# eichenberger/stereo-svo-slam

Hardware: AMD Instinct MI355X
Metric: tracked_frames_per_sec (higher is better)
Workload: dtype f32

## Files before the change

### include/svo_hip.h

```cpp
#ifndef SVO_HIP_H
#define SVO_HIP_H

#include <stddef.h>

#include "svo_types.h"

#ifdef __cplusplus
extern "C" {
#endif

enum {
    SVO_OK = 0,
    SVO_ERR_INVALID = -1,
    SVO_ERR_HIP = -2,
    SVO_ERR_NO_DEVICE = -3,
    SVO_ERR_CAPACITY = -4
};

typedef struct svo_handle svo_handle;

const char *svo_last_error(void);
int svo_version(void);

int svo_handle_create(int device, int max_keypoints, svo_handle **out);
// ... 621 lines not shown

typedef struct svo_voxel_map_info {
    float    voxel;
    int32_t  log2_capacity;
    uint32_t drop_flags;
    int32_t  _pad;
    int64_t  n_voxels;
    int64_t  n_fused;
    int64_t  n_outside;
    int64_t  overflow;
} svo_voxel_map_info;

typedef struct svo_voxel_filter {
    uint32_t min_count;
    uint32_t min_stamp;
    int32_t  _reserved[2];
} svo_voxel_filter;

int64_t svo_voxel_map_bytes(int log2_capacity);
int svo_voxel_clear(svo_handle *h, void *map, const svo_voxel_params *params);
int svo_voxel_fuse(svo_handle *h, int n_spans, const svo_voxel_span *spans, int n_maps, const svo_voxel_map *maps);
int svo_voxel_info(svo_handle *h, const void *map, svo_voxel_map_info *info);
int svo_voxel_extract(svo_handle *h, const svo_voxel_map *map, const svo_voxel_filter *filter, svo_map_point *points,
                      int64_t capacity, int64_t *n_points);

int svo_ctx_set_voxel_maps(svo_ctx *ctx, const int *seqs, int n, const svo_voxel_params *params);
int svo_get_voxel_map_info(svo_ctx *ctx, int seq, svo_voxel_map_info *info);

enum { SVO_FUSE_OK = 0, SVO_FUSE_NONE = 1, SVO_FUSE_NO_MAP = 2, SVO_FUSE_FULL = 3 };

typedef struct svo_fuse_info {
    int32_t seq, run;
    int32_t frame_id;
    int32_t keyframe_id;
    int32_t status;
    int32_t n_offered;
    int32_t n_fused, n_outside;
    int64_t n_voxels;
    float   pose[6];
} svo_fuse_info;

int svo_submit_fuse_clouds(svo_ctx *ctx, int what, const int *seqs, int n, const svo_cloud_style *style,
                           const svo_stereo_check *check, uint32_t stamp, svo_fuse_info *info);
int svo_fuse_clouds(svo_ctx *ctx, int what, const int *seqs, int n, const svo_cloud_style *style,
                    const svo_stereo_check *check, uint32_t stamp, svo_fuse_info *info);

enum { SVO_VOXEL_OK = 0, SVO_VOXEL_NO_MAP = 1, SVO_VOXEL_TOO_SMALL = 2 };

typedef struct svo_voxel_region {
    int64_t  first_point;
    int64_t  point_capacity;
    uint32_t min_stamp;
    int32_t  _reserved[3];
} svo_voxel_region;

typedef struct svo_voxel_segment {
    int32_t seq, run;
    int32_t frame_id;
    int32_t status;
    int64_t first_point;
    int64_t n_points;
    int64_t n_voxels;
    int64_t n_fused;
    float   voxel;
    int32_t log2_capacity;
    int64_t _pad;
} svo_voxel_segment;

typedef struct svo_voxel_dst {
    svo_voxel_segment *segments;
    svo_map_point     *points;
} svo_voxel_dst;

int svo_submit_export_voxel_maps(svo_ctx *ctx, const int *seqs, int n, const svo_voxel_region *regions,
                                 const svo_voxel_filter *filter, const svo_voxel_dst *dst, int mem);
int svo_export_voxel_maps(svo_ctx *ctx, const int *seqs, int n, const svo_voxel_region *regions,
                          const svo_voxel_filter *filter, const svo_voxel_dst *dst, int mem);
int svo_submit_clear_voxel_maps(svo_ctx *ctx, const int *seqs, int n);

#define SVO_SNAPSHOT_MAGIC   0x534f5653u
#define SVO_SNAPSHOT_VERSION 1
#define SVO_SNAPSHOT_BYTE_ORDER 0x01020304u
enum { SVO_SNAPSHOT_COMPLETE = 0,
       SVO_SNAPSHOT_TOO_SMALL = 1 };

struct svo_snapshot_info {
    uint32_t magic, version, byte_order;
    uint32_t status;
    int64_t  host_bytes, data_bytes;
    svo_camera_settings cam;
    int32_t  width, height;
    int32_t  capacity;
    int32_t  pyramid_levels, lk_levels;
    int32_t  frame_id;
    int32_t  n_keypoints;
    int32_t  n_trajectory;
    int32_t  n_keyframes, keyframes_retired;
    int32_t  n_image_sets;
    int32_t  n_planes;
    int32_t  first_keyframe;
};
typedef struct svo_snapshot_keyframe {
    float   pose[6];
    int32_t n;
    int32_t image_set;
} svo_snapshot_keyframe;
typedef struct svo_snapshot_plane {
    int64_t offset;
    int32_t row_bytes, rows;
} svo_snapshot_plane;

typedef struct svo_snapshot {
    void   *host;  int64_t host_capacity;
    void   *data;  int64_t data_capacity;
} svo_snapshot;

int svo_snapshot_size(svo_ctx *ctx, int seq, int64_t *host_bytes, int64_t *data_bytes);
int svo_submit_save(svo_ctx *ctx, const int *seqs, int n, svo_snapshot *snaps, int mem);
int svo_save_sequences(svo_ctx *ctx, const int *seqs, int n, svo_snapshot *snaps, int mem);
int svo_submit_load(svo_ctx *ctx, const int *seqs, int n, const svo_snapshot *snaps, int mem);
int svo_load_sequences(svo_ctx *ctx, const int *seqs, int n, const svo_snapshot *snaps, int mem);
int svo_snapshot_info(const void *host_part, int64_t bytes, struct svo_snapshot_info *out);
typedef struct svo_copy_segment {
    const void *src;
    void       *dst;
    int64_t     row_bytes, rows;
    int64_t     src_pitch, dst_pitch;
} svo_copy_segment;
int svo_copy_segments(svo_handle *h, int n, const svo_copy_segment *segs);

typedef struct svo_frame_stats {
    int32_t frame_id;
    int32_t is_keyframe;
    int32_t n_keypoints;
    int32_t n_keyframes;
    int32_t inside_count;
    int32_t overflow;
    float   pose_sia[6];
    float   pose_refined[6];
    float   sia_cost, reproj_cost;
    float   sia_ms;
    float   stage_ms[8];
    svo_gn_trace sia_trace[SVO_MAX_PYRAMID_LEVELS];
    svo_gn_trace reproj_trace;
} svo_frame_stats;
int svo_get_frame_stats(svo_ctx *ctx, int seq, svo_frame_stats *out);
typedef struct svo_totals {
    int64_t frames;
    int64_t keyframes;
    int64_t keypoints;
    int64_t gn_gradient_calls;
    int64_t gn_cost_calls;
    double  stage_ms[8];
    double  wall_ms;
    int64_t launches;
    int32_t n_groups;
    int32_t image_sets;
} svo_totals;
int svo_get_totals(svo_ctx *ctx, svo_totals *out);
int svo_ctx_enable_timing(svo_ctx *ctx, int on);
int svo_ctx_set_fast_solver(svo_ctx *ctx, int on);
int svo_ctx_set_exact_pinv(svo_ctx *ctx, int on);

enum { SVO_KERNEL_SIA_GN = 0,
       SVO_KERNEL_REPROJ_GN = 1 };
typedef struct svo_launch_shape {
    int32_t kernel;
    int32_t waves;
    int32_t mode;
    int32_t cap;
    int64_t launches;
} svo_launch_shape;
int svo_ctx_get_launch_shapes(svo_ctx *ctx, svo_launch_shape *out, int max, int *n);
int svo_pick_launch_shapes(const svo_camera_settings *cam, int width, int height, int batch, int n_bound,
                           int rec_cap, int exact, svo_launch_shape out[2]);
int svo_pick_sia_lds_bytes(const svo_camera_settings *cam, int width, int height, int batch, int n_bound,
                           int rec_cap, int exact, int64_t *lds_bytes);

int svo_pinv6_check(svo_handle *h, const float *H_dev, int n, float *out_dev, int32_t *sweeps_dev, int impl);
int svo_solve6_check(svo_handle *h, const float *H_dev, const float *b_dev, int n, float *out_dev,
                     int32_t *sweeps_dev, int impl);
int svo_sia_records_check(svo_handle *h, int batch, int stride, const int32_t *n_dev, int n_bound,
                          const svo_kp2d *kps2d, const uint32_t *flags, const svo_image *prev_pyr,
                          const svo_camera_settings *cam, int rec_cap, uint32_t ws_fill, float *rec_out,
                          float *ref_out, int64_t *n_diff, int64_t *first_diff);
int svo_reproj_gn_batch(svo_handle *h, int batch, int stride, const int32_t *n_dev, int n_bound, svo_kp2d *kps2d,
                        const svo_kp3d *kps3d, uint32_t *flags, const svo_camera_settings *cam,
                        const svo_kp2d *tracked, const float *err, const float *pose_in, float *pose_out,
                        float *cost, svo_gn_trace *trace, int32_t *zero_out, int *waves, int *cap);
int svo_sparse_align_batch(svo_handle *h, int batch, int stride, const int32_t *n_dev, int n_bound,
                           const svo_kp2d *kps2d, const svo_kp3d *kps3d, const uint32_t *flags,
                           const svo_image *prev_pyr, const svo_image *cur_pyr, const svo_camera_settings *cam,
                           const float *pose_guess, int dbg_level, uint32_t ws_fill, float *pose_out, float *cost,
                           svo_gn_trace *trace, float *dbg, int *waves, int *mode, int *cap);
int svo_sparse_align_batch_mats(svo_handle *h, int batch, int stride, const int32_t *n_dev, int n_bound,
                                const svo_kp2d *kps2d, const svo_kp3d *kps3d, const uint32_t *flags,
                                const svo_image *prev_pyr, const svo_image *cur_pyr, const svo_camera_settings *cam,
                                const float *pose_guess, int dbg_level, uint32_t ws_fill, float *pose_out, float *cost,
                                svo_gn_trace *trace, float *dbg, int *waves, int *mode, int *cap, void *mats_out);
int svo_pose_mats_layout(int64_t *block_bytes, int64_t *rd_offset, int64_t *r_offset, int64_t *ri_offset,
                         int64_t *t_offset);
int svo_filter_update_batch(svo_handle *h, int batch, int stride, const int32_t *n_dev, int n_bound, svo_kp2d *kps2d,
                            svo_kp3d *kps3d, uint32_t *flags, const svo_camera_settings *cam,
                            const float *frame_pose, const float *disparity, const svo_kp3d *ref3d,
                            const svo_kp2d *ref2d, const float *kf_pose, int32_t *outlier_count,
                            int32_t *inlier_count, float *kf_inv_depth, float *kf_variance,
                            int do_outlier_check, int do_update, int do_flags, int do_reproject, int width,
                            int height, int32_t *inside_count);
typedef struct svo_klt_keyframe {
    svo_image lk[SVO_LK_LEVELS];
    int32_t n_lk;
    int32_t n_kps;
    const svo_kp2d *kps2d;
    void *tmpl;
    uint8_t *tmpl_valid;
    int64_t tmpl_bytes, tmpl_valid_bytes;
    int32_t tmpl_cap, tmpl_win;
} svo_klt_keyframe;
typedef struct svo_klt_sequence {
    const svo_klt_keyframe *kfs;
    int32_t n_kfs;
    int32_t n_cur;
    svo_image cur[SVO_LK_LEVELS];
    const int32_t *n;
    const int32_t *kf_id;
    const int32_t *kp_index;
    const svo_kp3d *kps3d;
    const float *pose;
    svo_camera_settings cam;
    svo_kp2d *tracked;
    uint8_t *status;
    float *err;
    svo_kp2d *proj_out;
    svo_kp2d *ref_out;
} svo_klt_sequence;
int svo_klt_track_batch(svo_handle *h, int batch, const svo_klt_sequence *seqs, int n_bound, int win, int use_mats);
int svo_klt_cache_layout(int win, int64_t *record_bytes, int64_t *header_offset, int64_t *header_bytes, int *levels);

typedef struct svo_kps_planes {
    svo_kp2d *kps2d;
    svo_kp3d *kps3d;
    uint32_t *flags;
    int32_t  *kf_id, *kp_index, *outlier_count, *inlier_count;
    float    *kf_inv_depth, *kf_variance, *score;
    int32_t  *level_type;
    uint32_t *color;
    int32_t  *n;
} svo_kps_planes;
int svo_keyframe_launch_info(int cap, int max_cells, int tmpl_cap, int *compact_threads, int *merge_threads,
                             int64_t *tmpl_valid_bytes);
typedef struct svo_compact_sequence {
    svo_kps_planes src, dst;
    int32_t mode, width, height, start;
    const int32_t *enable;
    int32_t *zero, *zero_res, *min_kf;
    int32_t zero_count, zero_res_count;
} svo_compact_sequence;
int svo_compact_batch(svo_handle *h, int batch, const svo_compact_sequence *seqs, int cap, int *threads);
typedef struct svo_merge_sequence {
    svo_camera_settings cam;
    int32_t width, height;
    const svo_det_cell *det;
    const int32_t *n_det;
    svo_kps_planes kps;
    svo_det_cell *sel;
    int32_t *sel_level, *sel_cell, *occupied;
    int32_t *old_count, *overflow;
    const int32_t *enable;
    int32_t occupied_count, pad_;
} svo_merge_sequence;
int svo_keyframe_merge_batch(svo_handle *h, int batch, const svo_merge_sequence *seqs, int n_levels, int max_cells,
                             int cap, int *threads);
typedef struct svo_kf_init_sequence {
    svo_camera_settings cam;
    int32_t first_frame, new_kf_id, kf_mask, evict_id;
    svo_kps_planes kps, record;
    const int32_t *old_count;
    const float *disparity, *frame_pose;
    void *kfs;
    int64_t kfs_bytes;
    uint32_t *color_lcg;
    int32_t *n_out;
    const int32_t *enable;
    void *tmpl;
    uint8_t *tmpl_valid;
    int32_t tmpl_valid_bytes, tmpl_cap, tmpl_win, pad_;
} svo_kf_init_sequence;
int svo_keyframe_init_batch(svo_handle *h, int batch, const svo_kf_init_sequence *seqs, int cap);
int svo_keyframe_record_layout(int64_t *record_bytes, int64_t *n_offset, int64_t *pose_offset, int64_t *tmpl_offset,
                               int64_t *tmpl_valid_offset, int64_t *tmpl_cap_offset, int64_t *tmpl_win_offset,
                               int64_t plane_offsets[12]);
typedef struct svo_ssd_sequence {
    svo_image left, right;
    const int32_t *n;
    const svo_kp2d *kps2d;
    float *disparity;
    int32_t win, search_x, search_y, clamp_half;
    int32_t first, cap;
    const int32_t *first_ptr;
    const int32_t *enable;
} svo_ssd_sequence;
int svo_ssd_disparity_batch(svo_handle *h, int batch, const svo_ssd_sequence *seqs, int n_bound, int win, int search_y,
                            int *max_win);

typedef struct svo_filter_keyframe {
    float pose[6];
    svo_kp2d *kps2d;
    svo_kp3d *kps3d;
    uint32_t *flags;
    int32_t *outlier_count, *inlier_count;
    int32_t n, pad_;
} svo_filter_keyframe;
typedef struct svo_filter_table_sequence {
    svo_camera_settings cam;
    svo_kps_planes kps;
    const float *frame_pose;
    const float *disparity;
    const svo_filter_keyframe *kfs;
    void *records;
    int64_t records_bytes;
    int32_t table, kf_mask, width, height;
    int32_t *inside_count;
} svo_filter_table_sequence;
int svo_filter_update_table_batch(svo_handle *h, int batch, const svo_filter_table_sequence *seqs, int n_bound,
                                  int do_outlier_check, int do_update, int do_flags, int do_reproject);

#ifdef __cplusplus
}
#endif
#endif
```

### stereo-svo-slam_amd/csrc/depth.hip

```cpp
#include "svo_kernels.hpp"

namespace svo {

typedef uint32_t __attribute__((aligned(1))) u32_unaligned;
__device__ inline uint32_t load_u8x4(const ImgView& im, int y, int x, int valid) {
    const uint8_t* src = im.g() + (size_t)y * im.stride + x;
    uint32_t v;
    if (x + 4 <= im.w) {
        v = *reinterpret_cast<const u32_unaligned*>(src);
    } else {
        v = 0;
#pragma unroll
        for (int b = 0; b < 4; b++)
            if (x + b < im.w) v |= (uint32_t)src[b] << (8 * b);
    }
    if (valid < 4) v &= (1u << (8 * valid)) - 1u;
    return v;
}

__device__ inline uint4 load_u8x16(const ImgView& im, int y, int x, int valid, uint32_t flip, uint32_t pad) {
    uint32_t w[4];
    if (x + 16 <= im.w) {
        const uint8_t* src = im.g() + (size_t)y * im.stride + x;
        __builtin_memcpy(w, src, 16);
    } else {
#pragma unroll
        for (int k = 0; k < 4; k++) w[k] = load_u8x4(im, y, x + 4 * k, 4);
    }
#pragma unroll
    for (int k = 0; k < 4; k++) {
        const int nv = valid - 4 * k;
        const uint32_t vm = nv >= 4 ? 0xFFFFFFFFu : (nv <= 0 ? 0u : ((1u << (8 * nv)) - 1u));
        w[k] = ((w[k] ^ flip) & vm) | (pad & ~vm);
    }
    return make_uint4(w[0], w[1], w[2], w[3]);
}

constexpr int SSD_WIN_ALL = 35, SSD_MH_ALL = 17;
constexpr int SSD_MAX_MW = 65;
constexpr int SSD_T_STRIDE = 96;
constexpr int SSD_R_STRIDE = 144;
constexpr int SSD_W_STRIDE = 105;
#ifndef SVO_SSD_THREADS
#define SVO_SSD_THREADS 256
#endif
constexpr int SSD_THREADS = SVO_SSD_THREADS;

typedef int ssd_v4i __attribute__((ext_vector_type(4)));

template <int SSD_MAX_WIN, int SSD_MAX_MH>
__global__ __launch_bounds__(SSD_THREADS) void ssd_disparity_kernel(const SsdArgs* __restrict__ args) {
    constexpr int SSD_R_ROWS = SSD_MAX_WIN + SSD_MAX_MH, SSD_MAX_MATCH = SSD_MAX_MW * SSD_MAX_MH;
    const SsdArgs& a = args[blockIdx.y];
    if (a.enable && !*G(a.enable)) return;
    const int n = *G(a.n_ptr);
    const int kp = a.first + (a.first_ptr ? *G(a.first_ptr) : 0) + (int)blockIdx.x;
    if (kp >= n) return;
    const int tid = threadIdx.x, lane = tid & 63, wave = tid >> 6;

    __shared__ __attribute__((aligned(16))) uint8_t s_t[(SSD_MAX_WIN + 1) * SSD_T_STRIDE];
    __shared__ __attribute__((aligned(16))) uint8_t s_r[SSD_R_ROWS * SSD_R_STRIDE];
    __shared__ int s_w[SSD_MAX_MH * SSD_W_STRIDE];
    __shared__ int s_tt[4];
    __shared__ unsigned long long s_key[SSD_THREADS / 64];
    __shared__ int s_sum[SSD_THREADS / 64], s_cnt[SSD_THREADS / 64];

    const int window_before = a.win / 2, window_after = (a.win + 1) / 2;
    const int cols = a.left.w, rows = a.left.h;
    const svo_kp2d p = G(a.kps2d)[kp];
    const int x = (int)p.x, y = (int)p.y;
    const int x11 = max(0, x - window_before);
    const int x12 = min(cols - 1, x + window_after);
    const int y11 = max(0, y - window_before);
    const int y12 = min(rows, y + window_after);
    const int x21 = x11;
    const int x22 = min(cols - 1, x + window_after + a.search_x);
    const int y21 = max(0, y - window_before - a.search_y);
    const int y22 = min(rows - 1, y + window_after + a.search_y);
    const int tw = x12 - x11, th = y12 - y11, rw = x22 - x21, rh = y22 - y21;
    const int mw = rw - tw + 1, mh = rh - th + 1;
    bool skip = false;
    if (a.clamp_half && (x12 <= 0 || y12 <= 0 || x11 >= cols - 1 || y11 >= rows - 1)) skip = true;
    if (a.clamp_half && (x22 <= 0 || y22 <= 0 || x21 >= cols - 1 || y21 >= rows - 1)) skip = true;
    if (tw <= 0 || th <= 0 || mw <= 0 || mh <= 0) skip = true;
    if (tw > SSD_MAX_WIN || th > SSD_MAX_WIN || mw > SSD_MAX_MW || mh > SSD_MAX_MH || rw > SSD_W_STRIDE ||
        rh > SSD_R_ROWS)
        skip = true;
    if (skip) {
        if (tid == 0) G(a.disparity)[kp] = -1.0f;
        return;
    }

    static_assert(SSD_T_STRIDE % 16 == 0 && SSD_R_STRIDE % 16 == 0, "rows are whole 16-byte chunks");
    for (int i = tid; i < (SSD_MAX_WIN + 1) * (SSD_T_STRIDE / 16); i += SSD_THREADS) {
        const int r = i / (SSD_T_STRIDE / 16), ch = i % (SSD_T_STRIDE / 16);
        const int c = 16 * (ch - 1);
        uint4 v = make_uint4(0, 0, 0, 0);
        if (r < th && c >= 0 && c < tw) v = load_u8x16(a.left, y11 + r, x11 + c, tw - c, 0x80808080u, 0u);
        reinterpret_cast<uint4*>(s_t)[i] = v;
    }
    for (int i = tid; i < SSD_R_ROWS * (SSD_R_STRIDE / 16); i += SSD_THREADS) {
        const int r = i / (SSD_R_STRIDE / 16), ch = i % (SSD_R_STRIDE / 16);
        uint4 v = make_uint4(0, 0, 0, 0);
        if (r < rh && 16 * ch < rw) v = load_u8x16(a.right, y21 + r, x21 + 16 * ch, rw - 16 * ch, 0x80808080u, 0x80808080u);
        reinterpret_cast<uint4*>(s_r)[i] = v;
    }
    __syncthreads();

    if (wave == SSD_THREADS / 64 - 1) {
        int tt = 0;
        if (lane < th) {
            const uint32_t* trow = reinterpret_cast<const uint32_t*>(s_t + lane * SSD_T_STRIDE) + 4;
#pragma unroll
            for (int d = 0; d < 9; d++) tt = __builtin_amdgcn_sdot4((int)trow[d], (int)trow[d], tt, false);
        }
        tt = wave_sum_dpp_i(tt);
        if (lane == 0) s_tt[0] = tt;
    }
    if (tid < rw) {
        const int8_t* col = reinterpret_cast<const int8_t*>(s_r) + tid;
        int sq = 0;
        for (int r = 0; r < th; r++) {
            const int v = col[r * SSD_R_STRIDE];
            sq += __mul24(v, v);
        }
        s_w[tid] = sq;
        for (int k = 1; k < mh; k++) {
            const int vn = col[(k + th - 1) * SSD_R_STRIDE], vo = col[(k - 1) * SSD_R_STRIDE];
            sq += __mul24(vn, vn) - __mul24(vo, vo);
            s_w[k * SSD_W_STRIDE + tid] = sq;
        }
    }

    const int n_jb = (mw + 15) >> 4, n_mb = (mh + 15) >> 4;
    const int fm = lane & 15, fh = lane >> 4;
    constexpr int SSD_SLOTS = (10 + SSD_THREADS / 64 - 1) / (SSD_THREADS / 64);
    ssd_v4i acc[SSD_SLOTS];
    int task_of[SSD_SLOTS];
#pragma unroll
    for (int t = 0; t < SSD_SLOTS; t++) { acc[t] = ssd_v4i{0, 0, 0, 0}; task_of[t] = -1; }
    {
        int slot = 0;
        for (int task = wave; task < n_jb * n_mb && slot < SSD_SLOTS; task += SSD_THREADS / 64, slot++) {
            task_of[slot] = task;
            const int mb = task >= n_jb ? 1 : 0, jb = task - mb * n_jb;
            const int o = 16 + 16 * fh - fm;
            const uint32_t* tb = reinterpret_cast<const uint32_t*>(s_t) + (o >> 2);
            const unsigned sh = (unsigned)(o & 3);
            const uint8_t* ab = s_r + (16 * jb + 16 * fh);
            const int arow = 16 * mb + fm;
            ssd_v4i c = {0, 0, 0, 0};
            for (int r = 0; r < th; r++) {
                const uint32_t* t = tb + r * (SSD_T_STRIDE / 4);
                const uint32_t t0 = t[0], t1 = t[1], t2 = t[2], t3 = t[3], t4 = t[4];
                ssd_v4i bf;
                bf.x = (int)__builtin_amdgcn_alignbyte(t1, t0, sh);
                bf.y = (int)__builtin_amdgcn_alignbyte(t2, t1, sh);
                bf.z = (int)__builtin_amdgcn_alignbyte(t3, t2, sh);
                bf.w = (int)__builtin_amdgcn_alignbyte(t4, t3, sh);
                const ssd_v4i af = *reinterpret_cast<const ssd_v4i*>(ab + min(arow + r, SSD_R_ROWS - 1) * SSD_R_STRIDE);
                c = __builtin_amdgcn_mfma_i32_16x16x64_i8(af, bf, c, 0, 0, 0);
            }
            acc[slot] = c;
        }
    }
    __syncthreads();

    static_assert(sizeof(int) * SSD_MAX_MATCH <= SSD_R_ROWS * SSD_R_STRIDE, "match map must fit the region tile");
    static_assert(SSD_MAX_MH <= 32, "two row blocks of 16 at most");
    int* const s_m = reinterpret_cast<int*>(s_r);
    {
        const int seg_len = (mw + 7) >> 3;
        for (int item = tid; item < mh * 8; item += SSD_THREADS) {
            const int k = item >> 3, j0 = (item & 7) * seg_len, j1 = min(mw, j0 + seg_len);
            if (j0 < j1) {
                const int* wrow = &s_w[k * SSD_W_STRIDE];
                int sq = 0;
                for (int c = 0; c < tw; c++) sq += wrow[j0 + c];
                s_m[k * mw + j0] = sq;
                for (int j = j0 + 1; j < j1; j++) {
                    sq += wrow[j + tw - 1] - wrow[j - 1];
                    s_m[k * mw + j] = sq;
                }
            }
        }
    }
    __syncthreads();
    {
        const int stt = s_tt[0];
#pragma unroll
        for (int slot = 0; slot < SSD_SLOTS; slot++) {
            const int task = task_of[slot];
            if (task < 0) continue;
            const int mb = task >= n_jb ? 1 : 0, jb = task - mb * n_jb;
            const int j = 16 * jb + fm;
#pragma unroll
            for (int i = 0; i < 4; i++) {
                const int k = 16 * mb + 4 * fh + i;
                if (k < mh && j < mw) s_m[k * mw + j] += stt - 2 * acc[slot][i];
            }
        }
    }
    __syncthreads();

    const int nm = mw * mh;
    unsigned long long best = ~0ull;
    for (int o = tid; o < nm; o += SSD_THREADS) {
        const unsigned long long key = ((unsigned long long)__float_as_uint((float)s_m[o]) << 32) | (unsigned)o;
        best = key < best ? key : best;
    }
#pragma unroll
    for (int o = 32; o >= 1; o >>= 1) {
        const unsigned long long other = __shfl_xor(best, o, 64);
        best = other < best ? other : best;
    }
    if ((tid & 63) == 0) s_key[tid >> 6] = best;
    __syncthreads();
    best = s_key[0];
    for (int w = 1; w < SSD_THREADS / 64; w++) best = s_key[w] < best ? s_key[w] : best;
    const int min_o = (int)(best & 0xffffffffu);
    const int minx = min_o % mw, miny = min_o / mw;
    const float minVal = __uint_as_float((unsigned)(best >> 32));

    int sumj = 0, cnt = 0;
    const unsigned magic = ((1u << 20) + (unsigned)mw - 1u) / (unsigned)mw;
    for (int o = tid; o < nm; o += SSD_THREADS) {
        const int k = (int)(((unsigned)o * magic) >> 20), j = o - k * mw;
        if (j >= minx && k >= miny && (double)(float)s_m[o] <= (double)minVal) { sumj += j; cnt++; }
    }
    sumj = wave_sum_dpp_i(sumj);
    cnt = wave_sum_dpp_i(cnt);
    if ((tid & 63) == 0) { s_sum[tid >> 6] = sumj; s_cnt[tid >> 6] = cnt; }
    __syncthreads();
    if (tid == 0) {
        int ts = 0, tc = 0;
        for (int w = 0; w < SSD_THREADS / 64; w++) { ts += s_sum[w]; tc += s_cnt[w]; }
        float minPos = (float)ts;
        minPos = minPos / tc;
        G(a.disparity)[kp] = a.clamp_half ? fmaxf(0.5f, minPos) : minPos;
    }
}

int ssd_pick_max_win(int win, int search_y) { return win <= 31 && 2 * search_y + 1 <= 13 ? 31 : SSD_WIN_ALL; }

void launch_ssd(const SsdArgs* d_args, int batch, int max_n, int win, int search_y, hipStream_t stream) {
    if (max_n <= 0) return;
    if (ssd_pick_max_win(win, search_y) == 31)
        hipLaunchKernelGGL((ssd_disparity_kernel<31, 13>), dim3(max_n, batch), dim3(SSD_THREADS), 0, stream, d_args);
    else
        hipLaunchKernelGGL((ssd_disparity_kernel<SSD_WIN_ALL, SSD_MH_ALL>), dim3(max_n, batch), dim3(SSD_THREADS), 0, stream, d_args);
}

__global__ __launch_bounds__(64) void filter_update_kernel(const FilterArgs* __restrict__ args) {
    const FilterArgs& a = args[blockIdx.y];
    const int n = *G(a.n_ptr);
    if ((int)blockIdx.x * 64 >= n) return;
    const int tid = threadIdx.x;
    PoseMats s_frame;
    {
        float pose[6];
        for (int i = 0; i < 6; i++) pose[i] = G(a.frame_pose)[i];
        pose_mats(pose, s_frame);
    }
    const float fx = a.cam.fx, fy = a.cam.fy, cx = a.cam.cx, cy = a.cam.cy, baseline = a.cam.baseline;
    const CamD camd = make_camd(fx, fy, cx, cy, a.cam);
    int inside = 0;

    if (const int i = blockIdx.x * 64 + tid; i < n) {
        float kfp[6];
        svo_kp3d r3;
        svo_kp2d r2;
        SVO_GP(KfDev) kf = nullptr;
        int kidx = 0;
        if (a.kfs) {
            kf = &G(a.kfs)[G(a.kf_id)[i] & a.kf_mask];
            kidx = G(a.kp_index)[i];
            for (int q = 0; q < 6; q++) kfp[q] = kf->pose[q];
            r3 = G(kf->kps3d)[kidx];
            r2 = G(kf->kps2d)[kidx];
        } else {
            for (int q = 0; q < 6; q++) kfp[q] = G(a.kf_pose)[(size_t)i * 6 + q];
            r3 = svo_kp3d{0, 0, 0};
            r2 = svo_kp2d{0, 0};
            if (a.ref3d) r3 = G(a.ref3d)[i];
            if (a.ref2d) r2 = G(a.ref2d)[i];
        }
        PoseMats km;
        pose_mats(kfp, km);
        const svo_kp2d kp2 = G(a.kps2d)[i];
        uint32_t flags = G(a.flags)[i];
        int outl = G(a.outlier_count)[i], inl = G(a.inlier_count)[i];

        if (a.do_outlier_check) {
            const float d = G(a.disparity)[i];
            const float _z = baseline / (d < 0.5f ? 0.5f : d);
            const float _x = (kp2.x - cx) / fx * _z;
            const float _y = (kp2.y - cy) / fy * _z;
            float pw[3] = {_x, _y, _z};
            mat33f_vec(s_frame.R, pw, pw);
            pw[0] += s_frame.t[0]; pw[1] += s_frame.t[1]; pw[2] += s_frame.t[2];
            float av[3] = {pw[0] - kfp[0], pw[1] - kfp[1], pw[2] - kfp[2]};
            mat33f_vec(km.Ri, av, av);
            float rv[3] = {r3.x - kfp[0], r3.y - kfp[1], r3.z - kfp[2]};
            mat33f_vec(km.Ri, rv, rv);
            const float disp_ref = baseline / rv[2];
            const float disp = baseline / av[2];
            const float pixel_distance = disp - disp_ref;
            if (fabsf(pixel_distance) > 5 * 0.5f) outl++;
            else inl++;
        }

        svo_kp3d p3 = G(a.kps3d)[i];
        if (a.do_update) {
            const float c1[3] = {kfp[0], kfp[1], kfp[2]};
            const float c2[3] = {s_frame.t[0], s_frame.t[1], s_frame.t[2]};
            float diff[3] = {fabsf(c1[0] - c2[0]), fabsf(c1[1] - c2[1]), fabsf(c1[2] - c2[2])};
            mat33f_vec(km.Ri, diff, diff);
            if (flags & (SVO_IGNORE_COMPLETELY | SVO_IGNORE_DURING_REFINEMENT)) {
                outl++;
            } else if (!((double)diff[0] < 0.1 && (double)diff[1] < 0.1)) {
                float p1[3] = {r2.x - cx, r2.y - cy, fx};
                mat33f_vec(km.R, p1, p1);
                float p2[3] = {kp2.x - cx, kp2.y - cy, fx};
                mat33f_vec(s_frame.R, p2, p2);
                const float A[6] = {p1[0], -p2[0], p1[1], -p2[1], p1[2], -p2[2]};
                const float yv[3] = {c2[0] - c1[0], c2[1] - c1[1], c2[2] - c1[2]};
                float l[2];
                solve_svd_3x2(A, yv, l);
                const float deviation =
                    (float)(0.5 / (double)sqrtf(diff[0] * diff[0] + diff[1] * diff[1]));
                const float Rm = deviation * deviation;
                float Mx[9];
#pragma unroll
                for (int k = 0; k < 9; k++) Mx[k] = km.Ri[k] * l[0];
                const float pc[3] = {p1[0] - c1[0], p1[1] - c1[1], p1[2] - c1[2]};
                float new_p[3];
                mat33f_vec(Mx, pc, new_p);
                float _z = new_p[2];
                float kx = G(a.kf_inv_depth)[i], kP = G(a.kf_variance)[i];
                kf1_update(kx, kP, 0.0001f, Rm, 1 / _z);
                G(a.kf_inv_depth)[i] = kx;
                G(a.kf_variance)[i] = kP;
                _z = (float)(1.0 / (double)kx);
                const float _x = (r2.x - cx) / fx * _z;
                const float _y = (r2.y - cy) / fy * _z;
                float cp[3] = {_x, _y, _z};
                mat33f_vec(km.R, cp, cp);
                p3.x = c1[0] + cp[0];
                p3.y = c1[1] + cp[1];
                p3.z = c1[2] + cp[2];
            }
        }

        if (a.do_flags) {
            if (outl > inl) flags |= SVO_IGNORE_COMPLETELY;
            if (inl > outl) flags &= ~(uint32_t)SVO_IGNORE_TEMPORARY;
            if (kf) {
                G(kf->kps3d)[kidx] = p3;
                const uint32_t keep = G(kf->flags)[kidx] & SVO_IGNORE_DURING_REFINEMENT;
                G(kf->flags)[kidx] = keep | (flags & (SVO_IGNORE_TEMPORARY | SVO_IGNORE_COMPLETELY));
                G(kf->inlier_count)[kidx] = inl;
                G(kf->outlier_count)[kidx] = outl;
            }
        }
        G(a.kps3d)[i] = p3;
        if (a.do_flags) G(a.flags)[i] = flags;
        G(a.outlier_count)[i] = outl;
        G(a.inlier_count)[i] = inl;

        if (a.do_reproject) {
            const svo_kp2d q = project_point(s_frame.Rd, s_frame.t, camd, p3);
            G(a.kps2d)[i] = q;
            if (q.x > 0 && q.y > 0 && q.x < a.width && q.y < a.height && !(flags & SVO_IGNORE_COMPLETELY))
                inside++;
        }
    }
    if (a.inside_count) {
        inside = wave_sum_i(inside);
        if (tid == 0 && inside) atomicAdd(a.inside_count, inside);
    }
}

void launch_filter(const FilterArgs* d_args, int batch, int max_n, hipStream_t stream) {
    if (max_n <= 0) return;
    hipLaunchKernelGGL(filter_update_kernel, dim3((max_n + 63) / 64, batch), dim3(64), 0, stream, d_args);
}

}
```

### stereo-svo-slam_amd/csrc/svo_capi_check.hip

```cpp
#include <hip/hip_runtime.h>

#include <algorithm>
#include <climits>
#include <cstring>
#include <vector>

#include "svo_handle.hpp"

using namespace svo;

static bool bad_batch(int batch, const void* seqs) { return batch < 1 || batch > 4096 || !seqs; }

extern "C" int svo_pick_launch_shapes(const svo_camera_settings* cam, int width, int height, int batch, int n_bound,
                                      int rec_cap, int exact, svo_launch_shape out[2]) {
    if (!cam || !out || width < 1 || height < 1 || batch < 1)
        return svo_set_error(SVO_ERR_INVALID, "svo_pick_launch_shapes: bad arguments");
    const LaunchShape s = sia_pick_shape(batch, *cam, width, height, n_bound, rec_cap, exact);
    const LaunchShape r = reproj_pick_shape(batch, n_bound);
    out[0] = {SVO_KERNEL_SIA_GN, s.waves, s.mode, s.cap, s.fits ? 1 : 0};
    out[1] = {SVO_KERNEL_REPROJ_GN, r.waves, r.mode, r.cap, r.fits ? 1 : 0};
    return SVO_OK;
}

extern "C" int svo_pick_sia_lds_bytes(const svo_camera_settings* cam, int width, int height, int batch, int n_bound,
                                      int rec_cap, int exact, int64_t* lds_bytes) {
    if (!cam || !lds_bytes || width < 1 || height < 1 || batch < 1)
        return svo_set_error(SVO_ERR_INVALID, "svo_pick_sia_lds_bytes: bad arguments");
    *lds_bytes = (int64_t)sia_pick_shape(batch, *cam, width, height, n_bound, rec_cap, exact).lds;
    return SVO_OK;
}

template <int IMPL>
__global__ void __launch_bounds__(64) pinv6_check_kernel(const float* H, int n, float* out, int32_t* sweeps) {
    const long sys = IMPL == 0 ? (long)blockIdx.x * 64 + threadIdx.x : (long)blockIdx.x;
    if (sys >= n) return;
    const float* h = H + sys * 36;
    float At[6][6], W[6], Vt[6][6], Hinv[36];
#pragma unroll
    for (int i = 0; i < 6; i++)
#pragma unroll
        for (int j = 0; j < 6; j++) At[i][j] = h[j * 6 + i];
    const int sw = IMPL == 0 ? jacobi_svd6_reg(At, W, Vt) : jacobi_svd6_lanes(At, W, Vt);
    svd6_pinv(At, W, Vt, Hinv);
    if (IMPL == 1 && threadIdx.x != 0) return;
    float* o = out + sys * 114;
#pragma unroll
    for (int i = 0; i < 36; i++) o[i] = Hinv[i];
#pragma unroll
    for (int i = 0; i < 6; i++) o[36 + i] = W[i];
#pragma unroll
    for (int i = 0; i < 6; i++)
#pragma unroll
        for (int k = 0; k < 6; k++) { o[42 + i * 6 + k] = Vt[i][k]; o[78 + i * 6 + k] = At[i][k]; }
    sweeps[sys] = sw;
}

extern "C" int svo_pinv6_check(svo_handle* h, const float* H_dev, int n, float* out_dev, int32_t* sweeps_dev,
                               int impl) {
    CHECK_H(h);
    if (n < 0 || (n > 0 && (!H_dev || !out_dev || !sweeps_dev)) || (impl != 0 && impl != 1))
        return svo_set_error(SVO_ERR_INVALID, "svo_pinv6_check: bad arguments");
    if (n == 0) return SVO_OK;
    if (impl == 0)
        pinv6_check_kernel<0><<<(n + 63) / 64, 64, 0, h->stream>>>(H_dev, n, out_dev, sweeps_dev);
    else
        pinv6_check_kernel<1><<<n, 64, 0, h->stream>>>(H_dev, n, out_dev, sweeps_dev);
    HIP_TRY(hipGetLastError());
    return SVO_OK;
}

static int check_batch_counts(const char* who, int batch, int stride, const int32_t* n_dev, int n_bound) {
    if (bad_batch(batch, n_dev) || n_bound < 0 || stride < n_bound)
        return svo_set_error(SVO_ERR_INVALID, "%s: need 1 <= batch <= 4096, n_dev and 0 <= n_bound <= stride", who);
    std::vector<int32_t> n((size_t)batch);
    HIP_TRY(hipMemcpy(n.data(), n_dev, sizeof(int32_t) * (size_t)batch, hipMemcpyDeviceToHost));
    for (int b = 0; b < batch; b++)
        if (n[(size_t)b] < 0 || n[(size_t)b] > n_bound)
            return svo_set_error(SVO_ERR_INVALID, "%s: n_dev[%d] = %d is outside 0..n_bound = %d", who, b, n[(size_t)b], n_bound);
    return SVO_OK;
}

extern "C" int svo_reproj_gn_batch(svo_handle* h, int batch, int stride, const int32_t* n_dev, int n_bound, svo_kp2d* kps2d,
                                   const svo_kp3d* kps3d, uint32_t* flags, const svo_camera_settings* cam,
                                   const svo_kp2d* tracked, const float* err, const float* pose_in, float* pose_out,
                                   float* cost, svo_gn_trace* trace, int32_t* zero_out, int* waves, int* cap) {
    CHECK_H(h);
    if (!cam || !pose_in || !pose_out || (n_bound > 0 && (!kps2d || !kps3d || !flags)) || (!tracked != !err))
        return svo_set_error(SVO_ERR_INVALID, "svo_reproj_gn_batch: bad arguments");
    int rc = check_batch_counts("svo_reproj_gn_batch", batch, stride, n_dev, n_bound);
    if (rc) return rc;
    std::vector<ReprojArgs> blocks((size_t)batch);
    for (int b = 0; b < batch; b++) {
        ReprojArgs& ra = blocks[(size_t)b];
        const size_t o = (size_t)b * (size_t)stride;
        memset(&ra, 0, sizeof(ra));
        ra.cam = *cam;
        ra.n_ptr = n_dev + b;
        ra.kps2d = kps2d + o; ra.kps3d = kps3d + o; ra.flags = flags + o;
        ra.tracked = tracked ? tracked + o : nullptr; ra.err = err ? err + o : nullptr;
        ra.pose_in = pose_in + 6 * (size_t)b; ra.pose_out = pose_out + 6 * (size_t)b;
        ra.cost_out = cost ? cost + b : nullptr; ra.trace = trace ? trace + b : nullptr;
        ra.exact_pinv = h->exact_pinv;
        ra.zero_out = zero_out ? zero_out + b : nullptr;
    }
    ReprojArgs* d;
    rc = stage(h, blocks, &d);
    if (rc) return rc;
    const LaunchStatus st = launch_reproj(d, batch, n_bound, h->stream);
    HIP_TRY(st.err);
    if (waves) *waves = st.shape.waves;
    if (cap) *cap = st.shape.cap;
    if (!st.shape.fits) return svo_set_error(SVO_ERR_CAPACITY, "svo_reproj_gn_batch: %d keypoints do not fit LDS", n_bound);
    return finish_launch(h);
}

static int sparse_align_batch(svo_handle* h, int batch, int stride, const int32_t* n_dev, int n_bound,
                              const svo_kp2d* kps2d, const svo_kp3d* kps3d, const uint32_t* flags,
                              const svo_image* prev_pyr, const svo_image* cur_pyr,
                              const svo_camera_settings* cam, const float* pose_guess, int dbg_level,
                              uint32_t ws_fill, float* pose_out, float* cost, svo_gn_trace* trace, float* dbg,
                              int* waves, int* mode, int* cap, PoseMats* mats_out) {
    CHECK_H(h);
    if (!cam || !prev_pyr || !cur_pyr || !pose_guess || !pose_out || (n_bound > 0 && (!kps2d || !kps3d)))
        return svo_set_error(SVO_ERR_INVALID, "svo_sparse_align_batch: bad arguments");
    if (cam->max_pyramid_levels < 1 || cam->max_pyramid_levels > 7 || cam->min_pyramid_level_pose_estimation < 0 ||
        cam->min_pyramid_level_pose_estimation >= cam->max_pyramid_levels)
        return svo_set_error(SVO_ERR_INVALID, "svo_sparse_align_batch: max_pyramid_levels must be 1..7, min below it");
    if (cam->window_size_pose_estimator != 4)
        return svo_set_error(SVO_ERR_INVALID, "svo_sparse_align_batch: window_size_pose_estimator must be 4");
    int rc = check_batch_counts("svo_sparse_align_batch", batch, stride, n_dev, n_bound);
    if (rc) return rc;
    const int levels = cam->max_pyramid_levels;
    const int width = cur_pyr[0].width, height = cur_pyr[0].height;
    if (width < 1 || height < 1) return svo_set_error(SVO_ERR_INVALID, "svo_sparse_align_batch: cur_pyr[0] has no size");
    for (int b = 0; b < batch; b++)
        for (int l = cam->min_pyramid_level_pose_estimation; l < levels; l++) {
            const svo_image& p = prev_pyr[(size_t)b * levels + l];
            const svo_image& c = cur_pyr[(size_t)b * levels + l];
            if (!p.data || !c.data || p.width != (width >> l) || c.width != (width >> l) || p.height != (height >> l) ||
                c.height != (height >> l) || p.stride < p.width || c.stride < c.width)
                return svo_set_error(SVO_ERR_INVALID, "svo_sparse_align_batch: sequence %d level %d: every sequence needs "
                                     "images of one size, %d x %d at level 0", b, l, width, height);
        }
    const LaunchShape want = sia_pick_shape(batch, *cam, width, height, n_bound, INT_MAX, h->exact_pinv);
    if (waves) *waves = want.waves;
    if (mode) *mode = want.mode;
    if (cap) *cap = want.cap;
    if (!want.fits || want.cap > INT_MAX - 255)
        return svo_set_error(SVO_ERR_CAPACITY, "svo_sparse_align_batch: %d keypoints exceed the kernel's LDS", n_bound);
    const int rec_cap = (want.cap + 255) / 256 * 256;
    const size_t rec_floats = sia_rec_ws_floats(*cam, rec_cap), kp_floats = (size_t)9 * rec_cap;
    DevPtr<float> ws;
    HIP_TRY(dev_malloc(ws, sizeof(float) * (rec_floats + kp_floats) * (size_t)batch));
    HIP_TRY(hipMemsetD32Async(reinterpret_cast<hipDeviceptr_t>(ws.get()), (int)ws_fill,
                              (rec_floats + kp_floats) * (size_t)batch, h->stream));
    std::vector<SiaArgs> blocks((size_t)batch);
    for (int b = 0; b < batch; b++) {
        SiaArgs& sa = blocks[(size_t)b];
        const size_t o = (size_t)b * (size_t)stride;
        memset(&sa, 0, sizeof(sa));
        for (int l = cam->min_pyramid_level_pose_estimation; l < levels; l++) {
            sa.prev[l] = make_view(prev_pyr[(size_t)b * levels + l]);
            sa.cur[l] = make_view(cur_pyr[(size_t)b * levels + l]);
        }
        sa.cam = *cam;
        sa.n_ptr = n_dev + b;
        sa.kps2d = kps2d ? kps2d + o : nullptr; sa.kps3d = kps3d ? kps3d + o : nullptr;
        sa.flags = flags ? flags + o : nullptr;
        sa.pose_guess = pose_guess + 6 * (size_t)b; sa.pose_out = pose_out + 6 * (size_t)b;
        sa.cost_out = cost ? cost + b : nullptr;
        sa.trace = trace ? trace + (size_t)b * SVO_MAX_PYRAMID_LEVELS : nullptr;
        sa.rec_ws = ws.get() + (size_t)b * (rec_floats + kp_floats);
        sa.kp_ws = sa.rec_ws + rec_floats;
        sa.rec_cap = rec_cap;
        sa.dbg_H = dbg ? dbg + 48 * (size_t)b : nullptr; sa.dbg_level = dbg_level;
        sa.cap = stride;
        sa.exact_pinv = h->exact_pinv;
        sa.mats_out = mats_out ? mats_out + b : nullptr;
    }
    SiaArgs* d;
    rc = stage(h, blocks, &d);
    if (rc) return rc;
    const LaunchStatus st = launch_sia(d, batch, *cam, width, height, n_bound, rec_cap, h->exact_pinv, h->stream);
    HIP_TRY(st.err);
    if (!st.shape.fits) {
        (void)hipStreamSynchronize(h->stream);
        return svo_set_error(SVO_ERR_CAPACITY, "svo_sparse_align_batch: %d keypoints exceed the kernel's LDS or registers", n_bound);
    }
    HIP_TRY(hipGetLastError());
    HIP_TRY(hipStreamSynchronize(h->stream));
    return SVO_OK;
}

extern "C" int svo_sparse_align_batch(svo_handle* h, int batch, int stride, const int32_t* n_dev, int n_bound,
                                      const svo_kp2d* kps2d, const svo_kp3d* kps3d, const uint32_t* flags,
                                      const svo_image* prev_pyr, const svo_image* cur_pyr,
                                      const svo_camera_settings* cam, const float* pose_guess, int dbg_level,
                                      uint32_t ws_fill, float* pose_out, float* cost, svo_gn_trace* trace, float* dbg,
                                      int* waves, int* mode, int* cap) {
    return sparse_align_batch(h, batch, stride, n_dev, n_bound, kps2d, kps3d, flags, prev_pyr, cur_pyr, cam, pose_guess,
                              dbg_level, ws_fill, pose_out, cost, trace, dbg, waves, mode, cap, nullptr);
}

extern "C" int svo_sparse_align_batch_mats(svo_handle* h, int batch, int stride, const int32_t* n_dev, int n_bound,
                                           const svo_kp2d* kps2d, const svo_kp3d* kps3d, const uint32_t* flags,
                                           const svo_image* prev_pyr, const svo_image* cur_pyr,
                                           const svo_camera_settings* cam, const float* pose_guess, int dbg_level,
                                           uint32_t ws_fill, float* pose_out, float* cost, svo_gn_trace* trace, float* dbg,
                                           int* waves, int* mode, int* cap, void* mats_out) {
    if (!mats_out || (reinterpret_cast<uintptr_t>(mats_out) & (alignof(PoseMats) - 1)))
        return svo_set_error(SVO_ERR_INVALID, "svo_sparse_align_batch_mats: mats_out must be %zu-byte aligned device memory",
                             alignof(PoseMats));
    return sparse_align_batch(h, batch, stride, n_dev, n_bound, kps2d, kps3d, flags, prev_pyr, cur_pyr, cam, pose_guess,
                              dbg_level, ws_fill, pose_out, cost, trace, dbg, waves, mode, cap, static_cast<PoseMats*>(mats_out));
}

__global__ __launch_bounds__(64) void sia_prep_ref_kernel(const SiaArgs* __restrict__ args) {
    const SiaArgs& a = args[blockIdx.z];
    const int n = min(*G(a.n_ptr), a.rec_cap);
    const int level = a.cam.min_pyramid_level_pose_estimation + blockIdx.y;
    if (level >= a.cam.max_pyramid_levels) return;
    const int idx = blockIdx.x * 64 + threadIdx.x;
    const int kp = idx >> 4, px = idx & 15;
    const int span = (n + 3) & ~3;
    if (kp >= span) return;
    const ImgView prev = a.prev[level];
    const int divider = 1 << level;
    float g0 = 0, g1 = 0, psr = __builtin_nanf(""), i1 = __builtin_nanf("");
    const bool active = kp < n && !(a.flags && (G(a.flags)[kp] & SVO_IGNORE_TEMPORARY));
    if (active) {
        svo_kp2d kref = G(a.kps2d)[kp];
        if (level != 0) { kref.x /= divider; kref.y /= divider; }
        float kx = kref.x - 2.f, ky = kref.y - 2.f;
        for (int rr = 0; rr < (px >> 2); rr++) {
            kx += 1.f; kx += 1.f; kx += 1.f; kx += 1.f;
            kx -= 4.f;
            ky += 1.f;
        }
        for (int cc = 0; cc < (px & 3); cc++) kx += 1.f;
        if (!(((double)kx - 2.0) < 0 || ((double)ky - 2.0) < 0 ||
              ((double)kx + 3.0) >= prev.w || ((double)ky + 3.0) >= prev.h)) {
            const float int1 = patch_sum(prev.g(), prev.stride, kx + 1, ky);
            const float int2 = patch_sum(prev.g(), prev.stride, kx - 1, ky);
            const float int3 = patch_sum(prev.g(), prev.stride, kx, ky + 1);
            const float int4 = patch_sum(prev.g(), prev.stride, kx, ky - 1);
            g0 = int1 - int2; g1 = int3 - int4;
        }
        if (!(((double)kx - 1.0) < 0 || ((double)ky - 1.0) < 0 ||
              ((double)kx + 2.0) > prev.w || ((double)ky + 2.0) > prev.h))
            psr = patch_sum(prev.g(), prev.stride, kx, ky);
        const int ps = a.cam.window_size_pose_estimator;
        const float half_size = ((float)ps - 1.0f) / 2.0f;
        const float s1x = kref.x - half_size, s1y = kref.y - half_size;
        const float f1x = floorf(s1x), f1y = floorf(s1y);
        if (f1x >= 0.f && f1y >= 0.f && f1x < 65536.f && f1y < 65536.f) {
            const int ip1x = (int)f1x, ip1y = (int)f1y;
            if (ip1y + ps < prev.h && ip1x + ps < prev.w) {
                const float x12 = s1x - (float)ip1x, y12 = s1y - (float)ip1y;
                const float x11 = 1.0f - x12, y11 = 1.0f - y12;
                const float m0 = x11 * y11, m1 = x12 * y11, m2 = x11 * y12, m3 = x12 * y12;
                const uint8_t* p = prev.g() + (size_t)((px >> 2) + ip1y) * prev.stride + (px & 3) + ip1x;
                float t = 0;
                t += m0 * (float)p[0];
                t += m1 * (float)p[1];
                t += m2 * (float)p[prev.stride];
                t += m3 * (float)p[prev.stride + 1];
                i1 = t;
            }
        }
    }
    float* out = G(a.rec_ws) + (size_t)blockIdx.y * SIA_REC_ROWS * a.rec_cap;
    out[(size_t)(REC_I1 * 16 + px) * a.rec_cap + kp] = i1;
    out[(size_t)(REC_PS * 16 + px) * a.rec_cap + kp] = psr;
    out[(size_t)(REC_G0 * 16 + px) * a.rec_cap + kp] = g0;
    out[(size_t)(REC_G1 * 16 + px) * a.rec_cap + kp] = g1;
    const float gxx = row16_sum_dpp(g0 * g0), gxy = row16_sum_dpp(g0 * g1), gyy = row16_sum_dpp(g1 * g1);
    if (px == 0) {
        out[(size_t)64 * a.rec_cap + kp] = gxx;
        out[(size_t)65 * a.rec_cap + kp] = gxy;
        out[(size_t)66 * a.rec_cap + kp] = gyy;
    }
}

__global__ void __launch_bounds__(256) words_diff_kernel(const uint32_t* a, const uint32_t* b, size_t n, unsigned long long* out) {
    for (size_t i = (size_t)blockIdx.x * 256 + threadIdx.x; i < n; i += (size_t)gridDim.x * 256)
        if (a[i] != b[i]) {
            atomicAdd(&out[0], 1ull);
            atomicMin(&out[1], (unsigned long long)i);
        }
}

extern "C" int svo_sia_records_check(svo_handle* h, int batch, int stride, const int32_t* n_dev, int n_bound,
                                     const svo_kp2d* kps2d, const uint32_t* flags, const svo_image* prev_pyr,
                                     const svo_camera_settings* cam, int rec_cap, uint32_t ws_fill, float* rec_out,
                                     float* ref_out, int64_t* n_diff, int64_t* first_diff) {
    CHECK_H(h);
    if (!cam || !prev_pyr || !n_diff || !first_diff || (n_bound > 0 && !kps2d))
        return svo_set_error(SVO_ERR_INVALID, "svo_sia_records_check: bad arguments");
    if (cam->max_pyramid_levels < 1 || cam->max_pyramid_levels > 7 || cam->min_pyramid_level_pose_estimation < 0 ||
        cam->min_pyramid_level_pose_estimation >= cam->max_pyramid_levels)
        return svo_set_error(SVO_ERR_INVALID, "svo_sia_records_check: max_pyramid_levels must be 1..7, min below it");
    if (rec_cap < 4 || (rec_cap & 3) || rec_cap < n_bound || rec_cap > (1 << 20))
        return svo_set_error(SVO_ERR_INVALID, "svo_sia_records_check: rec_cap must be a multiple of 4 in n_bound..2^20");
    int rc = check_batch_counts("svo_sia_records_check", batch, stride, n_dev, n_bound);
    if (rc) return rc;
    const int levels = cam->max_pyramid_levels;
    for (int b = 0; b < batch; b++)
        for (int l = cam->min_pyramid_level_pose_estimation; l < levels; l++) {
            const svo_image& p = prev_pyr[(size_t)b * levels + l];
// ... 154 lines not shown
        }
    }
}

extern "C" int svo_solve6_check(svo_handle* h, const float* H_dev, const float* b_dev, int n, float* out_dev,
                                int32_t* sweeps_dev, int impl) {
    CHECK_H(h);
    if (n < 0 || (n > 0 && (!H_dev || !b_dev || !out_dev || !sweeps_dev)) || (impl != 0 && impl != 1))
        return svo_set_error(SVO_ERR_INVALID, "svo_solve6_check: bad arguments");
    if (n == 0) return SVO_OK;
    if (impl == 0)
        solve6_check_kernel<0><<<n, 64, 0, h->stream>>>(H_dev, b_dev, n, out_dev, sweeps_dev);
    else
        solve6_check_kernel<1><<<n, 64, 0, h->stream>>>(H_dev, b_dev, n, out_dev, sweeps_dev);
    HIP_TRY(hipGetLastError());
    return SVO_OK;
}

__global__ void klt_pose_mats_kernel(const float* const* poses, PoseMats* out) {
    pose_mats(poses[blockIdx.x], out[blockIdx.x]);
}

static_assert(sizeof(svo_klt_keyframe) == 128 && sizeof(svo_klt_sequence) == 248, "the layouts the Python binding restates");
static bool klt_bad_view(const svo_image& v) { return !v.data || v.width < 1 || v.height < 1 || v.stride < v.width; }

extern "C" int svo_klt_track_batch(svo_handle* h, int batch, const svo_klt_sequence* seqs, int n_bound, int win,
                                   int use_mats) {
    CHECK_H(h);
    if (bad_batch(batch, seqs) || n_bound < 0)
        return svo_set_error(SVO_ERR_INVALID, "svo_klt_track_batch: need 1 <= batch <= 4096, seqs and n_bound >= 0");
    if (win < 3 || win > 35) return svo_set_error(SVO_ERR_INVALID, "svo_klt_track_batch: window must be 3..35");
    HIP_TRY(hipStreamSynchronize(h->stream));
    const size_t rec_bytes = klt_template_bytes(win);
    std::vector<KfDev> table;
    std::vector<size_t> first_kf((size_t)batch);
    std::vector<int32_t> idx, ids;
    for (int b = 0; b < batch; b++) {
        const svo_klt_sequence& s = seqs[b];
        if (!s.kfs || s.n_kfs < 1 || s.n_kfs > 8 || s.n_cur < 1 || s.n_cur > SVO_LK_LEVELS || !s.n || !s.pose ||
            (n_bound > 0 && (!s.kp_index || !s.kps3d || !s.tracked || !s.status || !s.err || !s.proj_out)))
            return svo_set_error(SVO_ERR_INVALID, "svo_klt_track_batch: sequence %d: bad arguments", b);
        for (int l = 0; l < s.n_cur; l++)
            if (klt_bad_view(s.cur[l])) return svo_set_error(SVO_ERR_INVALID, "svo_klt_track_batch: sequence %d: current level %d", b, l);
        first_kf[(size_t)b] = table.size();
        for (int k = 0; k < s.n_kfs; k++) {
            const svo_klt_keyframe& f = s.kfs[k];
            if (f.n_lk < 1 || f.n_lk > SVO_LK_LEVELS || f.n_kps < 0 || (f.n_kps > 0 && !f.kps2d))
                return svo_set_error(SVO_ERR_INVALID, "svo_klt_track_batch: sequence %d keyframe %d: bad arguments", b, k);
            for (int l = 0; l < f.n_lk; l++)
                if (klt_bad_view(f.lk[l]))
                    return svo_set_error(SVO_ERR_INVALID, "svo_klt_track_batch: sequence %d keyframe %d: level %d", b, k, l);
            if (f.tmpl && f.tmpl_win == win) {
                const int64_t recs = (int64_t)f.tmpl_cap * SVO_LK_LEVELS;
                if (f.tmpl_cap < 0 || !f.tmpl_valid || f.tmpl_valid_bytes < recs || f.tmpl_bytes < recs * (int64_t)rec_bytes ||
                    (reinterpret_cast<uintptr_t>(f.tmpl) & 15))
                    return svo_set_error(SVO_ERR_INVALID, "svo_klt_track_batch: sequence %d keyframe %d: the cache needs %lld "
                                         "records of %zu bytes, 16-byte aligned, and as many flags", b, k, (long long)recs, rec_bytes);
            }
            KfDev kf;
            memset(&kf, 0, sizeof(kf));
            kf.n_lk = f.n_lk;
            for (int l = 0; l < f.n_lk; l++) kf.lk[l] = make_view(f.lk[l]);
            kf.kps2d = const_cast<svo_kp2d*>(f.kps2d);
            kf.n = f.n_kps;
            kf.tmpl = f.tmpl; kf.tmpl_valid = f.tmpl_valid; kf.tmpl_cap = f.tmpl_cap; kf.tmpl_win = f.tmpl_win;
            table.push_back(kf);
        }
        int32_t n = 0;
        HIP_TRY(hipMemcpy(&n, s.n, sizeof(n), hipMemcpyDeviceToHost));
        if (n < 0 || n > n_bound)
            return svo_set_error(SVO_ERR_INVALID, "svo_klt_track_batch: sequence %d: n = %d is outside 0..n_bound = %d", b, n, n_bound);
        idx.resize((size_t)n); ids.assign((size_t)n, 0);
        if (n > 0) {
            HIP_TRY(hipMemcpy(idx.data(), s.kp_index, sizeof(int32_t) * (size_t)n, hipMemcpyDeviceToHost));
            if (s.kf_id) HIP_TRY(hipMemcpy(ids.data(), s.kf_id, sizeof(int32_t) * (size_t)n, hipMemcpyDeviceToHost));
        }
        for (int i = 0; i < n; i++)
            if (ids[(size_t)i] < 0 || ids[(size_t)i] >= s.n_kfs || idx[(size_t)i] < 0 || idx[(size_t)i] >= s.kfs[ids[(size_t)i]].n_kps)
                return svo_set_error(SVO_ERR_INVALID, "svo_klt_track_batch: sequence %d point %d: keyframe %d, index %d", b, i,
                                     ids[(size_t)i], idx[(size_t)i]);
    }
    KfDev* d_table;
    int rc = stage(h, table, &d_table);
    if (rc) return rc;
    DevPtr<PoseMats> mats;
    if (use_mats) {
        std::vector<const float*> poses((size_t)batch);
        for (int b = 0; b < batch; b++) poses[(size_t)b] = seqs[b].pose;
        const float** d_poses;
        rc = stage(h, poses, &d_poses);
        if (rc) return rc;
        HIP_TRY(dev_malloc(mats, sizeof(PoseMats) * (size_t)batch));
        klt_pose_mats_kernel<<<batch, 1, 0, h->stream>>>(d_poses, mats.get());
        HIP_TRY(hipGetLastError());
    }
    std::vector<KltArgs> blocks((size_t)batch);
    for (int b = 0; b < batch; b++) {
        const svo_klt_sequence& s = seqs[b];
        KltArgs& ka = blocks[(size_t)b];
        memset(&ka, 0, sizeof(ka));
        ka.kfs = d_table + first_kf[(size_t)b]; ka.kf_mask = -1; ka.kf_id = s.kf_id; ka.n_cur = s.n_cur;
        for (int l = 0; l < s.n_cur; l++) ka.cur[l] = make_view(s.cur[l]);
        ka.n_ptr = s.n; ka.prev_pts = nullptr; ka.cur_pts = s.tracked; ka.status = s.status;
        ka.err = s.err; ka.win = win;
        ka.proj_pose = s.pose; ka.proj_mats = use_mats ? mats.get() + b : nullptr; ka.kps3d = s.kps3d; ka.proj_out = s.proj_out;
        ka.kp_index = s.kp_index; ka.ref_out = s.ref_out; ka.cam = s.cam;
    }
    KltArgs* d;
    rc = stage(h, blocks, &d);
    if (rc) { (void)hipStreamSynchronize(h->stream); return rc; }
    launch_klt(d, batch, n_bound, win, h->stream);
    return finish_launch(h);
}

extern "C" int svo_klt_cache_layout(int win, int64_t* record_bytes, int64_t* header_offset, int64_t* header_bytes, int* levels) {
    if (win < 3 || win > 35) return svo_set_error(SVO_ERR_INVALID, "svo_klt_cache_layout: window must be 3..35");
    if (record_bytes) *record_bytes = (int64_t)klt_template_bytes(win);
    if (header_offset) *header_offset = (int64_t)klt_template_header_offset(win);
    if (header_bytes) *header_bytes = (int64_t)klt_template_header_bytes();
    if (levels) *levels = SVO_LK_LEVELS;
    return SVO_OK;
}

static_assert(sizeof(svo_kps_planes) == 104 && sizeof(svo_compact_sequence) == 264 && sizeof(svo_merge_sequence) == 272 &&
              sizeof(svo_kf_init_sequence) == 400 && sizeof(svo_ssd_sequence) == 112, "the layouts the Python binding restates");

static KpsDev kps_dev(const svo_kps_planes& p) {
    KpsDev k;
    k.kps2d = p.kps2d; k.kps3d = p.kps3d; k.flags = p.flags; k.kf_id = p.kf_id; k.kp_index = p.kp_index;
    k.outl = p.outlier_count; k.inl = p.inlier_count; k.kfx = p.kf_inv_depth; k.kfP = p.kf_variance;
    k.score = p.score; k.level_type = p.level_type; k.color = p.color; k.n = p.n;
    return k;
}
static bool planes_missing(const svo_kps_planes& p, bool need_n) {
    return !p.kps2d || !p.kps3d || !p.flags || !p.kf_id || !p.kp_index || !p.outlier_count || !p.inlier_count ||
           !p.kf_inv_depth || !p.kf_variance || !p.score || !p.level_type || !p.color || (need_n && !p.n);
}
static int read_i32(const int32_t* dev, int count, int32_t* out) {
    HIP_TRY(hipMemcpy(out, dev, sizeof(int32_t) * (size_t)count, hipMemcpyDeviceToHost));
    return SVO_OK;
}

extern "C" int svo_keyframe_launch_info(int cap, int max_cells, int tmpl_cap, int* compact_threads, int* merge_threads,
                                        int64_t* tmpl_valid_bytes) {
    if (cap < 1 || max_cells < 1 || tmpl_cap < 0)
        return svo_set_error(SVO_ERR_INVALID, "svo_keyframe_launch_info: need cap >= 1, max_cells >= 1, tmpl_cap >= 0");
    if (compact_threads) *compact_threads = compact_pick_threads(cap);
    if (merge_threads) *merge_threads = select_merge_pick_threads(max_cells);
    if (tmpl_valid_bytes) *tmpl_valid_bytes = (int64_t)kf_tmpl_valid_bytes(tmpl_cap);
    return SVO_OK;
}

extern "C" int svo_compact_batch(svo_handle* h, int batch, const svo_compact_sequence* seqs, int cap, int* threads) {
    CHECK_H(h);
    if (bad_batch(batch, seqs) || cap < 1)
        return svo_set_error(SVO_ERR_INVALID, "svo_compact_batch: need 1 <= batch <= 4096, seqs and cap >= 1");
    HIP_TRY(hipStreamSynchronize(h->stream));
    std::vector<CompactArgs> blocks((size_t)batch);
    for (int b = 0; b < batch; b++) {
        const svo_compact_sequence& s = seqs[b];
        if (planes_missing(s.src, true) || planes_missing(s.dst, true) || (s.mode != 0 && s.mode != 1) ||
            (s.start != 0 && s.start != 1) || s.zero_count < 0 || s.zero_res_count < 0 || (s.zero_count > 0 && !s.zero) ||
            (s.zero_res_count > 0 && !s.zero_res))
            return svo_set_error(SVO_ERR_INVALID, "svo_compact_batch: sequence %d: bad arguments", b);
        if (s.min_kf && s.mode != 0)
            return svo_set_error(SVO_ERR_INVALID, "svo_compact_batch: sequence %d: min_kf is defined for mode 0 only", b);
        if (!s.start) {
            int32_t n = 0;
            if (const int rc = read_i32(s.src.n, 1, &n)) return rc;
            if (n < 0 || n > cap)
                return svo_set_error(SVO_ERR_INVALID, "svo_compact_batch: sequence %d: n = %d is outside 0..cap = %d", b, n, cap);
        }
        CompactArgs& ca = blocks[(size_t)b];
        memset(&ca, 0, sizeof(ca));
        ca.src = kps_dev(s.src); ca.dst = kps_dev(s.dst); ca.mode = s.mode;
        ca.width = s.width; ca.height = s.height;
        ca.enable = s.enable;
        ca.zero = s.zero; ca.zero_count = s.zero_count;
        ca.start = s.start;
        ca.zero_res = s.zero_res; ca.zero_res_count = s.zero_res_count;
        ca.min_kf = s.min_kf;
    }
    CompactArgs* d;
    const int rc = stage(h, blocks, &d);
    if (rc) return rc;
    if (threads) *threads = compact_pick_threads(cap);
    launch_compact(d, batch, cap, h->stream);
    return finish_launch(h);
}

extern "C" int svo_keyframe_merge_batch(svo_handle* h, int batch, const svo_merge_sequence* seqs, int n_levels,
                                        int max_cells, int cap, int* threads) {
    CHECK_H(h);
    if (bad_batch(batch, seqs) || n_levels < 1 || n_levels > SVO_MAX_PYRAMID_LEVELS || max_cells < 1 || cap < 1)
        return svo_set_error(SVO_ERR_INVALID, "svo_keyframe_merge_batch: need 1 <= batch <= 4096, seqs, n_levels 1..%d, "
                             "max_cells >= 1 and cap >= 1", SVO_MAX_PYRAMID_LEVELS);
    HIP_TRY(hipStreamSynchronize(h->stream));
    std::vector<MergeArgs> blocks((size_t)batch);
    for (int b = 0; b < batch; b++) {
        const svo_merge_sequence& s = seqs[b];
        if (planes_missing(s.kps, true) || !s.det || !s.n_det || !s.sel || !s.sel_level || !s.sel_cell || !s.occupied ||
            !s.old_count || !s.overflow || s.width < 1 || s.height < 1 || s.cam.grid_width < 1 || s.cam.grid_height < 1)
            return svo_set_error(SVO_ERR_INVALID, "svo_keyframe_merge_batch: sequence %d: bad arguments", b);
        const int64_t cells = ((int64_t)(s.width + s.cam.grid_height - 1) / s.cam.grid_height) *
                              ((int64_t)(s.height + s.cam.grid_width - 1) / s.cam.grid_width);
        if (cells > s.occupied_count)
            return svo_set_error(SVO_ERR_INVALID, "svo_keyframe_merge_batch: sequence %d: %lld merge cells, occupied holds %d", b,
                                 (long long)cells, s.occupied_count);
        int32_t nd[SVO_MAX_PYRAMID_LEVELS], n = 0;
        if (const int rc = read_i32(s.n_det, n_levels, nd)) return rc;
        if (const int rc = read_i32(s.kps.n, 1, &n)) return rc;
        for (int l = 0; l < n_levels; l++)
            if (nd[l] < 0 || nd[l] > max_cells)
                return svo_set_error(SVO_ERR_INVALID, "svo_keyframe_merge_batch: sequence %d: n_det[%d] = %d is outside "
                                     "0..max_cells = %d", b, l, nd[l], max_cells);
        if (n < 0 || n > cap)
            return svo_set_error(SVO_ERR_INVALID, "svo_keyframe_merge_batch: sequence %d: n = %d is outside 0..cap = %d", b, n, cap);
        MergeArgs& ma = blocks[(size_t)b];
        memset(&ma, 0, sizeof(ma));
        ma.cam = s.cam; ma.width = s.width; ma.height = s.height;
        ma.det = reinterpret_cast<const DetCell*>(s.det); ma.n_det = s.n_det; ma.n_levels = n_levels; ma.max_cells = max_cells;
        ma.kps = kps_dev(s.kps); ma.cap = cap;
        ma.sel = reinterpret_cast<DetCell*>(s.sel); ma.sel_level = s.sel_level; ma.sel_cell = s.sel_cell; ma.occupied = s.occupied;
        ma.old_count = s.old_count; ma.overflow = s.overflow;
        ma.enable = s.enable;
    }
    MergeArgs* d;
    const int rc = stage(h, blocks, &d);
    if (rc) return rc;
    if (threads) *threads = select_merge_pick_threads(max_cells);
    launch_select_merge(d, batch, max_cells, h->stream);
    return finish_launch(h);
}

extern "C" int svo_keyframe_record_layout(int64_t* record_bytes, int64_t* n_offset, int64_t* pose_offset, int64_t* tmpl_offset,
                                          int64_t* tmpl_valid_offset, int64_t* tmpl_cap_offset, int64_t* tmpl_win_offset,
                                          int64_t plane_offsets[12]) {
    if (record_bytes) *record_bytes = (int64_t)sizeof(KfDev);
    if (n_offset) *n_offset = (int64_t)offsetof(KfDev, n);
    if (pose_offset) *pose_offset = (int64_t)offsetof(KfDev, pose);
    if (tmpl_offset) *tmpl_offset = (int64_t)offsetof(KfDev, tmpl);
    if (tmpl_valid_offset) *tmpl_valid_offset = (int64_t)offsetof(KfDev, tmpl_valid);
    if (tmpl_cap_offset) *tmpl_cap_offset = (int64_t)offsetof(KfDev, tmpl_cap);
    if (tmpl_win_offset) *tmpl_win_offset = (int64_t)offsetof(KfDev, tmpl_win);
    if (plane_offsets) {
        const size_t o[12] = {offsetof(KfDev, kps2d), offsetof(KfDev, kps3d), offsetof(KfDev, flags), offsetof(KfDev, kf_id),
                              offsetof(KfDev, kp_index), offsetof(KfDev, outlier_count), offsetof(KfDev, inlier_count),
                              offsetof(KfDev, kfx), offsetof(KfDev, kfP), offsetof(KfDev, score), offsetof(KfDev, level_type),
                              offsetof(KfDev, color)};
        for (int i = 0; i < 12; i++) plane_offsets[i] = (int64_t)o[i];
    }
    return SVO_OK;
}

extern "C" int svo_keyframe_init_batch(svo_handle* h, int batch, const svo_kf_init_sequence* seqs, int cap) {
    CHECK_H(h);
    if (bad_batch(batch, seqs) || cap < 1)
        return svo_set_error(SVO_ERR_INVALID, "svo_keyframe_init_batch: need 1 <= batch <= 4096, seqs and cap >= 1");
    HIP_TRY(hipStreamSynchronize(h->stream));
    std::vector<KfInitArgs> blocks((size_t)batch);
    for (int b = 0; b < batch; b++) {
        const svo_kf_init_sequence& s = seqs[b];
        if (planes_missing(s.kps, true) || planes_missing(s.record, false) || !s.old_count || !s.disparity || !s.kfs ||
            !s.color_lcg || !s.n_out || (!s.first_frame && !s.frame_pose) || (s.first_frame != 0 && s.first_frame != 1) ||
            s.new_kf_id < 0 || s.evict_id < -1)
            return svo_set_error(SVO_ERR_INVALID, "svo_keyframe_init_batch: sequence %d: bad arguments", b);
        if (s.kf_mask < 0 || s.kf_mask > (1 << 20) || ((s.kf_mask + 1) & s.kf_mask) != 0 ||
            (int64_t)(s.kf_mask + 1) * (int64_t)sizeof(KfDev) > s.kfs_bytes || (reinterpret_cast<uintptr_t>(s.kfs) & 7))
            return svo_set_error(SVO_ERR_INVALID, "svo_keyframe_init_batch: sequence %d: the table needs kf_mask + 1 = a power "
                                 "of two records of %zu bytes, 8-byte aligned", b, sizeof(KfDev));
        if (s.tmpl_valid_bytes < 0 || s.tmpl_valid_bytes % 4 != 0 || (s.tmpl_valid_bytes > 0 && !s.tmpl_valid) ||
            (reinterpret_cast<uintptr_t>(s.tmpl_valid) & 3))
            return svo_set_error(SVO_ERR_INVALID, "svo_keyframe_init_batch: sequence %d: tmpl_valid must be 4-byte aligned and "
                                 "tmpl_valid_bytes a multiple of 4", b);
        int32_t n = 0, old_count = 0;
        if (const int rc = read_i32(s.kps.n, 1, &n)) return rc;
        if (const int rc = read_i32(s.old_count, 1, &old_count)) return rc;
        if (n < 0 || n > cap || old_count < 0 || old_count > n)
            return svo_set_error(SVO_ERR_INVALID, "svo_keyframe_init_batch: sequence %d: need 0 <= old_count = %d <= n = %d <= "
                                 "cap = %d", b, old_count, n, cap);
        KfInitArgs& ia = blocks[(size_t)b];
        memset(&ia, 0, sizeof(ia));
        ia.cam = s.cam; ia.kps = kps_dev(s.kps); ia.old_count = s.old_count;
        ia.disparity = s.disparity; ia.frame_pose = s.frame_pose;
        ia.first_frame = s.first_frame; ia.new_kf_id = s.new_kf_id; ia.kfs = static_cast<KfDev*>(s.kfs); ia.kf_mask = s.kf_mask;
        ia.color_lcg = s.color_lcg; ia.n_out = s.n_out;
        ia.enable = s.enable;
        KfDev& r = ia.record;
        r.kps2d = s.record.kps2d; r.kps3d = s.record.kps3d; r.flags = s.record.flags;
        r.outlier_count = s.record.outlier_count; r.inlier_count = s.record.inlier_count;
        r.kf_id = s.record.kf_id; r.kp_index = s.record.kp_index; r.score = s.record.score;
        r.level_type = s.record.level_type; r.color = s.record.color; r.kfx = s.record.kf_inv_depth; r.kfP = s.record.kf_variance;
        r.tmpl = s.tmpl; r.tmpl_valid = s.tmpl_valid; r.tmpl_cap = s.tmpl_cap; r.tmpl_win = s.tmpl_win;
        ia.tmpl_valid_bytes = s.tmpl_valid_bytes;
        ia.evict_id = s.evict_id;
    }
    KfInitArgs* d;
    const int rc = stage(h, blocks, &d);
    if (rc) return rc;
    launch_kf_init(d, batch, h->stream);
    return finish_launch(h);
}

extern "C" int svo_ssd_disparity_batch(svo_handle* h, int batch, const svo_ssd_sequence* seqs, int n_bound, int win,
                                       int search_y, int* max_win) {
    CHECK_H(h);
    constexpr int kMaxIndex = 1 << 29;
    if (bad_batch(batch, seqs) || n_bound < 0 || n_bound > kMaxIndex)
        return svo_set_error(SVO_ERR_INVALID, "svo_ssd_disparity_batch: need 1 <= batch <= 4096, seqs and 0 <= n_bound <= 2^29");
    if (win < 1 || win > 35 || search_y < 0 || search_y > 8)
        return svo_set_error(SVO_ERR_INVALID, "svo_ssd_disparity_batch: win<=35, search_y<=8 supported");
    HIP_TRY(hipStreamSynchronize(h->stream));
    std::vector<SsdArgs> blocks((size_t)batch);
    for (int b = 0; b < batch; b++) {
        const svo_ssd_sequence& s = seqs[b];
        if (klt_bad_view(s.left) || klt_bad_view(s.right) || !s.n || s.cap < 0 || (s.cap > 0 && (!s.kps2d || !s.disparity)) ||
            s.first < 0 || s.first > kMaxIndex)
            return svo_set_error(SVO_ERR_INVALID, "svo_ssd_disparity_batch: sequence %d: bad arguments", b);
        if (s.win < 1 || s.win > win || s.search_x < 0 || s.search_x > 64 || s.search_y < 0 || s.search_y > search_y)
            return svo_set_error(SVO_ERR_INVALID, "svo_ssd_disparity_batch: sequence %d: win %d, search_x %d, search_y %d exceed "
                                 "the launch's %d, 64, %d", b, s.win, s.search_x, s.search_y, win, search_y);
        int32_t n = 0, first = 0;
        if (const int rc = read_i32(s.n, 1, &n)) return rc;
        if (s.first_ptr)
            if (const int rc = read_i32(s.first_ptr, 1, &first)) return rc;
        if (n < 0 || n > s.cap || first < 0 || first > kMaxIndex)
            return svo_set_error(SVO_ERR_INVALID, "svo_ssd_disparity_batch: sequence %d: n = %d is outside 0..cap = %d, or "
                                 "*first_ptr = %d is outside 0..2^29", b, n, s.cap, first);
        SsdArgs& sa = blocks[(size_t)b];
        memset(&sa, 0, sizeof(sa));
        sa.left = make_view(s.left); sa.right = make_view(s.right);
        sa.n_ptr = s.n; sa.kps2d = s.kps2d; sa.disparity = s.disparity;
        sa.win = s.win; sa.search_x = s.search_x; sa.search_y = s.search_y; sa.clamp_half = s.clamp_half;
        sa.first = s.first; sa.first_ptr = s.first_ptr;
        sa.enable = s.enable;
    }
    SsdArgs* d;
    const int rc = stage(h, blocks, &d);
    if (rc) return rc;
    if (max_win) *max_win = ssd_pick_max_win(win, search_y);
    launch_ssd(d, batch, n_bound, win, search_y, h->stream);
    return finish_launch(h);
}

static_assert(sizeof(svo_filter_keyframe) == 72 && sizeof(svo_filter_table_sequence) == 248, "the layouts the Python binding restates");

extern "C" int svo_filter_update_table_batch(svo_handle* h, int batch, const svo_filter_table_sequence* seqs, int n_bound,
                                             int do_outlier_check, int do_update, int do_flags, int do_reproject) {
    CHECK_H(h);
    if (bad_batch(batch, seqs) || n_bound < 0)
        return svo_set_error(SVO_ERR_INVALID, "svo_filter_update_table_batch: need 1 <= batch <= 4096, seqs and n_bound >= 0");
    HIP_TRY(hipStreamSynchronize(h->stream));
    std::vector<std::vector<KfDev>> tables((size_t)batch);
    std::vector<int32_t> ids, idx;
    for (int b = 0; b < batch; b++) {
        const svo_filter_table_sequence& s = seqs[b];
        const svo_kps_planes& p = s.kps;
        if (!s.kfs || !s.records || !s.frame_pose || !p.n || !p.kps2d || !p.kps3d || !p.flags || !p.kf_id || !p.kp_index ||
            !p.outlier_count || !p.inlier_count || !p.kf_inv_depth || !p.kf_variance || (do_outlier_check && !s.disparity))
            return svo_set_error(SVO_ERR_INVALID, "svo_filter_update_table_batch: sequence %d: bad arguments", b);
        const bool ring = s.kf_mask != -1;
        if (s.table < 1 || s.table > 4096 || (ring && ((s.table & (s.table - 1)) != 0 || s.kf_mask != s.table - 1)) ||
            (int64_t)s.table * (int64_t)sizeof(KfDev) > s.records_bytes || (reinterpret_cast<uintptr_t>(s.records) & 7))
            return svo_set_error(SVO_ERR_INVALID, "svo_filter_update_table_batch: sequence %d: the table needs 1..4096 records "
                                 "of %zu bytes, 8-byte aligned; a ring (kf_mask != -1) a power of two of them and kf_mask = "
                                 "table - 1", b, sizeof(KfDev));
        std::vector<KfDev>& rec = tables[(size_t)b];
        rec.resize((size_t)s.table);
        for (int k = 0; k < s.table; k++) {
            const svo_filter_keyframe& f = s.kfs[k];
            if (f.n < 0 || (f.n > 0 && (!f.kps2d || !f.kps3d || !f.flags || !f.outlier_count || !f.inlier_count)))
                return svo_set_error(SVO_ERR_INVALID, "svo_filter_update_table_batch: sequence %d keyframe %d: bad arguments", b, k);
            KfDev& d = rec[(size_t)k];
            memset(&d, 0, sizeof(d));
            memcpy(d.pose, f.pose, sizeof(d.pose));
            d.kps2d = f.kps2d; d.kps3d = f.kps3d; d.flags = f.flags;
            d.outlier_count = f.outlier_count; d.inlier_count = f.inlier_count;
            d.n = f.n;
        }
        int32_t n = 0;
        if (const int rc = read_i32(p.n, 1, &n)) return rc;
        if (n < 0 || n > n_bound)
            return svo_set_error(SVO_ERR_INVALID, "svo_filter_update_table_batch: sequence %d: n = %d is outside 0..n_bound = %d",
                                 b, n, n_bound);
        ids.resize((size_t)n); idx.resize((size_t)n);
        if (n > 0) {
            if (const int rc = read_i32(p.kf_id, n, ids.data())) return rc;
            if (const int rc = read_i32(p.kp_index, n, idx.data())) return rc;
        }
        for (int i = 0; i < n; i++) {
            const int slot = ids[(size_t)i] & s.kf_mask;
            if (ids[(size_t)i] < 0 || slot >= s.table || idx[(size_t)i] < 0 || idx[(size_t)i] >= s.kfs[slot].n)
                return svo_set_error(SVO_ERR_INVALID, "svo_filter_update_table_batch: sequence %d point %d: keyframe %d, index %d",
                                     b, i, ids[(size_t)i], idx[(size_t)i]);
        }
    }
    std::vector<FilterArgs> blocks((size_t)batch);
    for (int b = 0; b < batch; b++) {
        const svo_filter_table_sequence& s = seqs[b];
        HIP_TRY(hipMemcpy(s.records, tables[(size_t)b].data(), sizeof(KfDev) * (size_t)s.table, hipMemcpyHostToDevice));
        FilterArgs& fa = blocks[(size_t)b];
        memset(&fa, 0, sizeof(fa));
        fill_filter_table_args(fa, s.cam, kps_dev(s.kps), s.frame_pose, s.disparity, static_cast<KfDev*>(s.records), s.kf_mask,
                               s.width, s.height, s.inside_count);
        fa.do_outlier_check = do_outlier_check; fa.do_update = do_update; fa.do_flags = do_flags; fa.do_reproject = do_reproject;
    }
    FilterArgs* d;
    const int rc = stage(h, blocks, &d);
    if (rc) return rc;
    launch_filter(d, batch, n_bound, h->stream);
    return finish_launch(h);
}
```

### stereo-svo-slam_amd/stereo_svo_slam_amd/hip_lib.py

```python
import ctypes as C
import os

import numpy as np
import torch

_HERE = os.path.dirname(os.path.abspath(__file__))
CSRC = os.path.normpath(os.path.join(_HERE, "..", "csrc"))
LIB_PATH = os.environ.get("SVO_HIP_LIB", os.path.join(CSRC, "libsvo_hip.so"))
_LIB = None

SYMBOLS = (
    "svo_last_error", "svo_version", "svo_handle_create", "svo_handle_destroy",
    "svo_handle_set_stream", "svo_handle_synchronize", "svo_build_pyramid",
    "svo_build_lk_pyramid", "svo_sparse_align", "svo_klt_track", "svo_reproj_gn",
    "svo_ssd_disparity", "svo_depth_filter_update",
    "svo_ctx_create", "svo_ctx_destroy", "svo_new_images", "svo_submit_images", "svo_wait",
    "svo_ctx_get_groups", "svo_new_image", "svo_get_pose",
    "svo_get_frame_keypoints", "svo_get_keyframe_count", "svo_get_keyframe",
    "svo_get_trajectory", "svo_update_pose", "svo_get_frame_stats", "svo_ctx_enable_timing",
    "svo_get_totals", "svo_handle_set_exact_pinv", "svo_ctx_set_exact_pinv",
    "svo_handle_set_fast_solver", "svo_ctx_set_fast_solver",
    "svo_device_malloc", "svo_device_free", "svo_copy_to_device", "svo_copy_to_host",
    "svo_copy_image_to_device", "svo_project_keypoints",
    "svo_ctx_get_launch_shapes", "svo_pick_launch_shapes", "svo_pick_sia_lds_bytes", "svo_pinv6_check",
    "svo_solve6_check", "svo_remap_linear", "svo_ctx_set_rectification",
    "svo_detect_keypoints", "svo_detect_shape",
    "svo_ctx_restart_sequences", "svo_get_finished_runs", "svo_get_finished_run",
    "svo_drop_finished_runs", "svo_ctx_get_memory",
    "svo_input_format_info", "svo_convert_frames", "svo_ctx_set_input_format",
    "svo_export_capacity", "svo_submit_export", "svo_export", "svo_pack_keypoints",
    "svo_snapshot_size", "svo_submit_save", "svo_save_sequences", "svo_submit_load", "svo_load_sequences",
    "svo_snapshot_info", "svo_copy_segments",
    "svo_reproj_gn_batch", "svo_filter_update_batch", "svo_sparse_align_batch",
    "svo_submit_pose_updates", "svo_update_poses", "svo_pose_filter_batch",
    "svo_map_size", "svo_submit_export_map", "svo_export_map", "svo_pack_map_points",
    "svo_view_size", "svo_submit_export_views", "svo_export_views", "svo_render_views",
    "svo_disparity_size", "svo_submit_export_disparity", "svo_export_disparity", "svo_dense_disparity",
    "svo_cloud_size", "svo_submit_export_cloud", "svo_export_cloud", "svo_cloud_points",
    "svo_disparity_size_checked", "svo_submit_export_disparity_checked", "svo_export_disparity_checked",
    "svo_dense_disparity_checked", "svo_submit_export_cloud_checked", "svo_export_cloud_checked",
    "svo_cloud_points_checked",
    "svo_scene_size", "svo_scene_look_at", "svo_scene_frustum", "svo_submit_export_scenes", "svo_export_scenes",
    "svo_render_scene",
    "svo_submit_export_scenes_clouds", "svo_export_scenes_clouds", "svo_render_scene_clouds",
    "svo_voxel_map_bytes", "svo_voxel_clear", "svo_voxel_fuse", "svo_voxel_info", "svo_voxel_extract",
    "svo_ctx_set_voxel_maps", "svo_get_voxel_map_info", "svo_submit_fuse_clouds", "svo_fuse_clouds",
    "svo_submit_export_voxel_maps", "svo_export_voxel_maps", "svo_submit_clear_voxel_maps",
    "svo_ar_size", "svo_ar_camera_of_pose", "svo_submit_export_ar", "svo_export_ar", "svo_render_ar",
    "svo_remap_linear_multi", "svo_ctx_add_rigs", "svo_ctx_remove_rigs", "svo_ctx_assign_rigs", "svo_ctx_get_slot_rig",
    "svo_ctx_get_rigs",
    "svo_klt_track_batch", "svo_klt_cache_layout",
    "svo_rectify_inverse", "svo_build_rectify_maps", "svo_ctx_add_rigs_calibrated", "svo_ctx_set_calibration",
    "svo_submit_trim_keyframes", "svo_trim_keyframes", "svo_ctx_set_keyframe_window", "svo_get_keyframe_range",
    "svo_keyframe_launch_info", "svo_compact_batch", "svo_keyframe_merge_batch", "svo_keyframe_init_batch",
    "svo_keyframe_record_layout", "svo_ssd_disparity_batch",
    "svo_sparse_align_batch_mats", "svo_pose_mats_layout", "svo_filter_update_table_batch",
    "svo_sia_records_check",
)

INPUT_GRAY_PAIR, INPUT_BGR_PAIR, INPUT_RGB_PAIR, INPUT_SBS_GRAY, INPUT_SBS_BGR, INPUT_SBS_RGB, INPUT_CH3_ECON = range(7)
INPUT_FORMATS = ("gray_pair", "bgr_pair", "rgb_pair", "sbs_gray", "sbs_bgr", "sbs_rgb", "ch3_econ")
INGEST_COPY, INGEST_GRAY = 0, 1
EXPORT_FRAMES, EXPORT_LAST_KEYFRAMES = 0, 1
EXPORT_WHAT = ("frames", "last_keyframes")
MEM_HOST, MEM_DEVICE = 0, 1


class SvoError(RuntimeError):
    pass


class CameraSettings(C.Structure):
    _fields_ = [(n, C.c_float) for n in
                ("baseline", "fx", "fy", "cx", "cy", "k1", "k2", "k3", "p1", "p2")] + \
               [(n, C.c_int32) for n in
                ("grid_height", "grid_width", "search_x", "search_y",
                 "window_size_pose_estimator", "window_size_opt_flow",
                 "window_size_depth_calculator", "max_pyramid_levels",
                 "min_pyramid_level_pose_estimation")]

    @classmethod
    def from_dict(cls, d):
        cam = cls()
        for name, _ in cls._fields_:
            setattr(cam, name, d[name])
        return cam


RIG_FLOATS = ("baseline", "fx", "fy", "cx", "cy", "k1", "k2", "k3", "p1", "p2")


class Rig(C.Structure):
    _fields_ = [(n, C.c_float) for n in RIG_FLOATS] + \
               [(n, C.c_void_p) for n in ("left_map_x", "left_map_y", "right_map_x", "right_map_y")] + \
               [("mem", C.c_int32), ("_reserved", C.c_int32)]

    @classmethod
    def from_dict(cls, d):
        get = d.__getitem__ if isinstance(d, dict) else lambda n: getattr(d, n)
        return cls(**{n: get(n) for n in RIG_FLOATS})


assert C.sizeof(Rig) == 80


class CameraCalibration(C.Structure):
    _fields_ = [("K", C.c_double * 9), ("D", C.c_double * 8), ("R", C.c_double * 9), ("P", C.c_double * 9)]

    @classmethod
    def from_mats(cls, K, D, R, P):
        K, P = np.asarray(K, np.float64), np.asarray(P, np.float64)
        D = np.asarray(D, np.float64).ravel()
        R = np.eye(3) if R is None else np.asarray(R, np.float64)
        if K.shape != (3, 3) or R.shape != (3, 3) or P.shape not in ((3, 3), (3, 4)):
            raise ValueError(f"K, R are 3x3 and P is 3x3 or 3x4, not {K.shape}, {R.shape}, {P.shape}")
        if D.size not in (4, 5, 8):
            raise ValueError(f"D has 4, 5 or 8 coefficients, not {D.size}")
        cal = cls()
        cal.K[:] = K.ravel().tolist()
        cal.D[:] = D.tolist() + [0.0] * (8 - D.size)
        cal.R[:] = R.ravel().tolist()
        cal.P[:] = P[:, :3].ravel().tolist()
        return cal


assert C.sizeof(CameraCalibration) == 280


class Image(C.Structure):
    _fields_ = [("data", C.c_void_p), ("width", C.c_int32), ("height", C.c_int32),
                ("stride", C.c_int32)]


class KltKeyframe(C.Structure):
    _fields_ = [("lk", Image * 3), ("n_lk", C.c_int32), ("n_kps", C.c_int32), ("kps2d", C.c_void_p),
                ("tmpl", C.c_void_p), ("tmpl_valid", C.c_void_p), ("tmpl_bytes", C.c_int64),
                ("tmpl_valid_bytes", C.c_int64), ("tmpl_cap", C.c_int32), ("tmpl_win", C.c_int32)]


class KltSequence(C.Structure):
    _fields_ = [("kfs", C.POINTER(KltKeyframe)), ("n_kfs", C.c_int32), ("n_cur", C.c_int32), ("cur", Image * 3),
                ("n", C.c_void_p), ("kf_id", C.c_void_p), ("kp_index", C.c_void_p), ("kps3d", C.c_void_p),
                ("pose", C.c_void_p), ("cam", CameraSettings)] + \
               [(n, C.c_void_p) for n in ("tracked", "status", "err", "proj_out", "ref_out")]


assert (C.sizeof(KltKeyframe), C.sizeof(KltSequence)) == (128, 248)


KPS_PLANES = ("kps2d", "kps3d", "flags", "kf_id", "kp_index", "outlier_count", "inlier_count", "kf_inv_depth",
              "kf_variance", "score", "level_type", "color", "n")


class KpsPlanes(C.Structure):
    _fields_ = [(name, C.c_void_p) for name in KPS_PLANES]


class CompactSequence(C.Structure):
    _fields_ = [("src", KpsPlanes), ("dst", KpsPlanes), ("mode", C.c_int32), ("width", C.c_int32), ("height", C.c_int32),
                ("start", C.c_int32), ("enable", C.c_void_p), ("zero", C.c_void_p), ("zero_res", C.c_void_p),
                ("min_kf", C.c_void_p), ("zero_count", C.c_int32), ("zero_res_count", C.c_int32)]


class MergeSequence(C.Structure):
    _fields_ = [("cam", CameraSettings), ("width", C.c_int32), ("height", C.c_int32), ("det", C.c_void_p),
                ("n_det", C.c_void_p), ("kps", KpsPlanes), ("sel", C.c_void_p), ("sel_level", C.c_void_p),
                ("sel_cell", C.c_void_p), ("occupied", C.c_void_p), ("old_count", C.c_void_p), ("overflow", C.c_void_p),
                ("enable", C.c_void_p), ("occupied_count", C.c_int32), ("pad_", C.c_int32)]


class KfInitSequence(C.Structure):
    _fields_ = [("cam", CameraSettings), ("first_frame", C.c_int32), ("new_kf_id", C.c_int32), ("kf_mask", C.c_int32),
                ("evict_id", C.c_int32), ("kps", KpsPlanes), ("record", KpsPlanes), ("old_count", C.c_void_p),
                ("disparity", C.c_void_p), ("frame_pose", C.c_void_p), ("kfs", C.c_void_p), ("kfs_bytes", C.c_int64),
                ("color_lcg", C.c_void_p), ("n_out", C.c_void_p), ("enable", C.c_void_p), ("tmpl", C.c_void_p),
                ("tmpl_valid", C.c_void_p), ("tmpl_valid_bytes", C.c_int32), ("tmpl_cap", C.c_int32),
                ("tmpl_win", C.c_int32), ("pad_", C.c_int32)]


class SsdSequence(C.Structure):
    _fields_ = [("left", Image), ("right", Image), ("n", C.c_void_p), ("kps2d", C.c_void_p), ("disparity", C.c_void_p),
                ("win", C.c_int32), ("search_x", C.c_int32), ("search_y", C.c_int32), ("clamp_half", C.c_int32),
                ("first", C.c_int32), ("cap", C.c_int32), ("first_ptr", C.c_void_p), ("enable", C.c_void_p)]


class FilterKeyframe(C.Structure):
    _fields_ = [("pose", C.c_float * 6)] + \
               [(n, C.c_void_p) for n in ("kps2d", "kps3d", "flags", "outlier_count", "inlier_count")] + \
               [("n", C.c_int32), ("pad_", C.c_int32)]


class FilterTableSequence(C.Structure):
    _fields_ = [("cam", CameraSettings), ("kps", KpsPlanes), ("frame_pose", C.c_void_p), ("disparity", C.c_void_p),
                ("kfs", C.POINTER(FilterKeyframe)), ("records", C.c_void_p), ("records_bytes", C.c_int64),
                ("table", C.c_int32), ("kf_mask", C.c_int32), ("width", C.c_int32), ("height", C.c_int32),
                ("inside_count", C.c_void_p)]


assert (C.sizeof(KpsPlanes), C.sizeof(CompactSequence), C.sizeof(MergeSequence), C.sizeof(KfInitSequence),
        C.sizeof(SsdSequence), C.sizeof(FilterKeyframe), C.sizeof(FilterTableSequence)) == (104, 264, 272, 400, 112, 72, 248)


def _addr(x):
    if x is None:
        return None
    if isinstance(x, int):
        return C.c_void_p(x)
    assert x.is_cuda
    return C.c_void_p(x.data_ptr())


def _fill(struct, d, skip=()):
    for name, typ in struct._fields_:
        if name in skip or name not in d or d[name] is None:
            continue
        v = d[name]
        if typ is C.c_void_p:
            setattr(struct, name, _addr(v))
        elif typ is KpsPlanes:
            _fill(getattr(struct, name), v)
        elif typ in (C.c_int32, C.c_int64):
            setattr(struct, name, int(v))
        else:
            setattr(struct, name, v)


class InputSide(C.Structure):
    _fields_ = [("buffer", C.c_int32), ("start_column", C.c_int32), ("op", C.c_int32), ("channel", C.c_int32),
                ("weight", C.c_int32 * 3)]


class InputLayout(C.Structure):
    _fields_ = [("buffers", C.c_int32), ("channels", C.c_int32), ("min_row_pixels", C.c_int32),
                ("left", InputSide), ("right", InputSide)]


GN_TRACE_DTYPE = np.dtype([("level", "<i4"), ("n_gradient", "<i4"), ("n_cost", "<i4"),
                           ("n_accepted", "<i4"), ("exit_small", "<i4"),
                           ("initial_cost", "<f4"), ("final_cost", "<f4"), ("pose", "<f4", (6,))])
assert GN_TRACE_DTYPE.itemsize == 52


DET_CELL_DTYPE = np.dtype([("x", "<f4"), ("y", "<f4"), ("score", "<f4"), ("type", "<i4")])
assert DET_CELL_DTYPE.itemsize == 16


EXPORT_SEGMENT_DTYPE = np.dtype([("seq", "<i4"), ("run", "<i4"), ("frame_id", "<i4"), ("keyframe_id", "<i4"),
                                 ("is_keyframe", "<i4"), ("n", "<i4"), ("first", "<i8"), ("pose", "<f4", (6,)),
                                 ("time_stamp", "<f4"), ("_pad", "<i4")])
assert EXPORT_SEGMENT_DTYPE.itemsize == 64


class ExportDst(C.Structure):
    _fields_ = [("segments", C.c_void_p), ("kps2d", C.c_void_p), ("kps3d", C.c_void_p), ("info", C.c_void_p),
                ("capacity", C.c_int64)]


MAP_POINT_DTYPE = np.dtype([("x", "<f4"), ("y", "<f4"), ("z", "<f4"), ("color", "u1", (3,)), ("flags", "u1")])
MAP_KEYFRAME_DTYPE = np.dtype([("id", "<i4"), ("n_total", "<i4"), ("n", "<i4"), ("_pad", "<i4"), ("first", "<i8"),
                               ("pose", "<f4", (6,))])
MAP_SEGMENT_DTYPE = np.dtype([("seq", "<i4"), ("run", "<i4"), ("frame_id", "<i4"), ("status", "<i4"),
                              ("n_keyframes", "<i4"), ("keyframes_retired", "<i4"), ("from_keyframe", "<i4"),
                              ("n_exported", "<i4"), ("n_points", "<i8"), ("points_bound", "<i8"),
                              ("time_stamp", "<f4"), ("_pad", "<i4", (3,))])
MAP_REGION_DTYPE = np.dtype([("first_point", "<i8"), ("point_capacity", "<i8"), ("first_keyframe_entry", "<i8"),
                             ("keyframe_capacity", "<i4"), ("from_keyframe", "<i4")])
assert (MAP_POINT_DTYPE.itemsize, MAP_KEYFRAME_DTYPE.itemsize, MAP_SEGMENT_DTYPE.itemsize,
        MAP_REGION_DTYPE.itemsize) == (16, 48, 64, 32)
MAP_COMPLETE, MAP_TOO_SMALL = 0, 1


def map_first_keyframe(segment):
    return int(segment["_pad"][0])
IGNORE_DURING_REFINEMENT, IGNORE_COMPLETELY, IGNORE_TEMPORARY = 1, 2, 4


class MapFilter(C.Structure):
    _fields_ = [("drop_flags", C.c_uint32), ("own_only", C.c_int32), ("min_inliers", C.c_int32),
                ("_reserved", C.c_int32)]


class MapDst(C.Structure):
    _fields_ = [("segments", C.c_void_p), ("keyframes", C.c_void_p), ("points", C.c_void_p)]


def map_filter(f):
    if f is None:
        return MapFilter()
    return f if isinstance(f, MapFilter) else MapFilter(**f)


PLANE_LEFT, PLANE_RIGHT = 0, 1
PLANES = ("left", "right")
PIXEL_GRAY8, PIXEL_RGB8, PIXEL_RGBA8 = 0, 1, 2
PIXELS = ("gray8", "rgb8", "rgba8")
PIXEL_BYTES = (1, 3, 4)
VIEW_OK, VIEW_NONE = 0, 1
VIEW_SEGMENT_DTYPE = np.dtype([("seq", "<i4"), ("run", "<i4"), ("frame_id", "<i4"), ("keyframe_id", "<i4"),
                               ("status", "<i4"), ("n", "<i4"), ("offset", "<i8"), ("pose", "<f4", (6,)),
                               ("time_stamp", "<f4"), ("_pad", "<i4")])
assert VIEW_SEGMENT_DTYPE.itemsize == 64


class ViewStyle(C.Structure):
    _fields_ = [("plane", C.c_int32), ("level", C.c_int32), ("pixel", C.c_int32), ("markers", C.c_int32),
                ("drop_flags", C.c_uint32), ("size", C.c_int32), ("size_temporary", C.c_int32),
                ("_reserved", C.c_int32)]


class ViewDst(C.Structure):
    _fields_ = [("segments", C.c_void_p), ("pixels", C.c_void_p), ("capacity", C.c_int64)]


def view_style(what=EXPORT_FRAMES, plane=PLANE_LEFT, level=0, pixel=PIXEL_GRAY8, markers=False, drop_flags=None,
               size=None, size_temporary=None):
    if isinstance(plane, str):
        plane = PLANES.index(plane)
    if isinstance(pixel, str):
        pixel = PIXELS.index(pixel)
    frames = int(what) == EXPORT_FRAMES
    return ViewStyle(int(plane), int(level), int(pixel), int(bool(markers)),
                     (IGNORE_COMPLETELY if frames else 0) if drop_flags is None else int(drop_flags),
                     (20 if frames else 10) if size is None else int(size),
                     10 if size_temporary is None else int(size_temporary), 0)


def view_size(cam, width, height, style):
    cols, rows, pitch, nbytes = C.c_int(0), C.c_int(0), C.c_int64(0), C.c_int64(0)
    _check(lib().svo_view_size(C.byref(cam), int(width), int(height), C.byref(style), C.byref(cols), C.byref(rows),
                               C.byref(pitch), C.byref(nbytes)))
    return cols.value, rows.value, pitch.value, nbytes.value


class Keypoints(C.Structure):
    _fields_ = [("n", C.c_int32)] + [(name, C.c_void_p) for name in (
        "kps2d", "kps3d", "flags", "keyframe_id", "keypoint_index", "outlier_count", "inlier_count",
        "kf_inv_depth", "kf_variance", "score", "level_type", "color")]


class ViewSrc(C.Structure):
    _fields_ = [("image", Image), ("kps", Keypoints)]


DENSE_DISPARITY, DENSE_DEPTH = 0, 1
DENSE_VALUES = ("disparity", "depth")
DISPARITY_OK, DISPARITY_NONE = 0, 1
DISPARITY_SEGMENT_DTYPE = np.dtype([("seq", "<i4"), ("run", "<i4"), ("frame_id", "<i4"), ("keyframe_id", "<i4"),
                                    ("status", "<i4"), ("_pad", "<i4"), ("offset", "<i8"), ("pose", "<f4", (6,)),
                                    ("time_stamp", "<f4"), ("baseline", "<f4")])
assert DISPARITY_SEGMENT_DTYPE.itemsize == 64


class DisparityStyle(C.Structure):
    _fields_ = [("value", C.c_int32), ("step", C.c_int32), ("win", C.c_int32), ("search_x", C.c_int32),
                ("search_y", C.c_int32), ("cost", C.c_int32), ("_reserved", C.c_int32 * 2)]


class DisparitySegment(C.Structure):
    _fields_ = [("seq", C.c_int32), ("run", C.c_int32), ("frame_id", C.c_int32), ("keyframe_id", C.c_int32),
                ("status", C.c_int32), ("_pad", C.c_int32), ("offset", C.c_int64), ("pose", C.c_float * 6),
# ... 746 lines not shown
        cams = (SceneCamera * max(n, 1))(*cameras)
        keep = []
        for i, (cols, rows, sets, lines) in enumerate(srcs):
            ks = (Keypoints * max(len(sets), 1))()
            own = (C.c_int32 * max(len(sets), 1))()
            for j, (m, own_id, planes) in enumerate(sets):
                ks[j].n, own[j] = int(m), int(own_id)
                for name, v in planes.items():
                    setattr(ks[j], name, v.data_ptr() if isinstance(v, torch.Tensor) else int(v))
            keep += [ks, own]
            n_lines = 0 if lines is None else lines.numel() * lines.element_size() // SCENE_LINE_DTYPE.itemsize
            arr[i] = SceneSrc(int(cols), int(rows), len(sets), n_lines, C.cast(ks, C.c_void_p), C.cast(own, C.c_void_p),
                              lines.data_ptr() if n_lines else None)
        offs = (C.c_int64 * max(n, 1))(*[int(o) for o in offsets])
        return n, arr, cams, offs, keep

    def render_scene_packed(self, packed, style, pixels):
        n, arr, cams, offs, _ = packed
        p = pixels.data_ptr() if isinstance(pixels, torch.Tensor) else int(pixels)
        _check(lib().svo_render_scene(self._h, n, arr, cams, offs, C.byref(style), C.c_void_p(p)))

    def render_scene_clouds(self, srcs, spans, cameras, offsets, style, point_size, pixels):
        packed = self.pack_scene(srcs, cameras, offsets)
        self.render_scene_clouds_packed(packed, self.pack_scene_spans(spans), style, point_size, pixels)

    def pack_scene_spans(self, spans):
        flat = [scene_span(e) for per_image in spans for e in per_image]
        arr = (SceneSpan * max(len(flat), 1))(*flat)
        counts = (C.c_int32 * max(len(spans), 1))(*[len(per_image) for per_image in spans])
        return arr, counts, spans

    def render_scene_clouds_packed(self, packed, packed_spans, style, point_size, pixels):
        n, arr, cams, offs, _ = packed
        p = pixels.data_ptr() if isinstance(pixels, torch.Tensor) else int(pixels)
        _check(lib().svo_render_scene_clouds(self._h, n, arr, packed_spans[0], packed_spans[1], cams, offs, C.byref(style),
                                             C.c_int32(int(point_size)), C.c_void_p(p)))

    def render_ar(self, srcs, cameras, offsets, style, pixels):
        self.render_ar_packed(self.pack_ar(srcs, cameras, offsets), style, pixels)

    def pack_ar(self, srcs, cameras, offsets):
        n = len(srcs)
        arr = (ArSrc * max(n, 1))()
        cams = (ArCamera * max(n, 1))(*cameras)
        keep = []
        for i, (img, draws) in enumerate(srcs):
            data, w, h, stride = img
            ds = (ArDraw * max(len(draws), 1))()
            for j, (model, vertices, triangles, rgb, rgb_all) in enumerate(draws):
                ds[j] = ArDraw((C.c_float * 12)(*[float(x) for x in np.asarray(model).ravel()]), vertices.data_ptr(),
                               triangles.data_ptr(), None if rgb is None else rgb.data_ptr(), vertices.numel() // 3,
                               triangles.numel() // 3, int(rgb_all), 0)
            keep.append(ds)
            arr[i] = ArSrc(Image(data.data_ptr() if isinstance(data, torch.Tensor) else int(data), int(w), int(h), int(stride)),
                           C.cast(ds, C.c_void_p), len(draws), 0)
        offs = (C.c_int64 * max(n, 1))(*[int(o) for o in offsets])
        return n, arr, cams, offs, keep

    def render_ar_packed(self, packed, style, pixels):
        n, arr, cams, offs, _ = packed
        p = pixels.data_ptr() if isinstance(pixels, torch.Tensor) else int(pixels)
        _check(lib().svo_render_ar(self._h, n, arr, cams, offs, C.byref(style), C.c_void_p(p)))

    def copy_segments(self, segs):
        arr = (CopySegment * max(len(segs), 1))(*[CopySegment(*[int(x) for x in g]) for g in segs])
        _check(lib().svo_copy_segments(self._h, len(segs), arr))

    def pose_filter_batch(self, state_in, start_pose, first, samples, state_out, filtered=None):
        b, total = state_in.shape[0], samples.shape[0]
        assert state_in.shape == (b, POSE_FILTER_IN_FLOATS) and state_out.shape == (b, POSE_FILTER_OUT_FLOATS)
        assert start_pose.shape == (b, 6) and first.shape == (b + 1,) and first.dtype == torch.int32
        assert samples.dtype == torch.uint8 and samples.shape == (total, POSE_SAMPLE_DTYPE.itemsize)
        assert filtered is None or filtered.shape == (total, 6)
        for t in (state_in, start_pose, state_out, filtered):
            assert t is None or t.dtype == torch.float32
        _check(lib().svo_pose_filter_batch(self._h, b, _ptr(state_in), _ptr(start_pose), _ptr(first), total,
                                           _ptr(samples), _ptr(state_out), _ptr(filtered)))

    def build_lk_pyramid(self, img, win, max_levels=3):
        levels = [img]
        h, w = img.shape
        for _ in range(1, max_levels):
            h = (h + 1) // 2
            w = (w + 1) // 2
            levels.append(torch.empty((h, w), dtype=torch.uint8, device=img.device))
        arr = _imgs(levels)
        n = C.c_int(0)
        _check(lib().svo_build_lk_pyramid(self._h, max_levels, win, arr, C.byref(n)))
        return levels[:n.value]

    def sparse_align(self, prev_pyr, cur_pyr, kps2d, kps3d, flags, cam, pose_guess,
                     dbg_level=-1):
        dev = kps2d.device
        n = kps2d.shape[0]
        pose_out = torch.zeros(6, dtype=torch.float32, device=dev)
        cost = torch.zeros(1, dtype=torch.float32, device=dev)
        trace = torch.zeros(8 * GN_TRACE_DTYPE.itemsize, dtype=torch.uint8, device=dev)
        dbg = torch.zeros(48, dtype=torch.float32, device=dev) if dbg_level >= 0 else None
        _check(lib().svo_sparse_align(
            self._h, _imgs(prev_pyr, 8), _imgs(cur_pyr, 8), _ptr(kps2d), _ptr(kps3d), _ptr(flags),
            n, C.byref(cam), _ptr(pose_guess), _ptr(pose_out), _ptr(cost), _ptr(trace), _ptr(dbg),
            dbg_level))
        return pose_out, cost, trace, dbg

    def sparse_align_batch(self, n, n_bound, kps2d, kps3d, flags, prev_pyrs, cur_pyrs, cam, pose_guess, dbg_level=-1,
                           ws_fill=0, outputs=None, mats_out=None):
        batch, stride = kps2d.shape[0], kps2d.shape[1]
        dev = kps2d.device
        levels = cam.max_pyramid_levels
        if outputs is None:
            outputs = (torch.zeros((batch, 6), dtype=torch.float32, device=dev),
                       torch.zeros(batch, dtype=torch.float32, device=dev),
                       torch.zeros((batch, 8 * GN_TRACE_DTYPE.itemsize), dtype=torch.uint8, device=dev),
                       torch.zeros((batch, 48), dtype=torch.float32, device=dev) if dbg_level >= 0 else None)
        pose_out, cost, trace, dbg = outputs
        pp, cp = (Image * (batch * levels))(), (Image * (batch * levels))()
        for b in range(batch):
            for l in range(levels):
                pp[b * levels + l], cp[b * levels + l] = _img(prev_pyrs[b][l]), _img(cur_pyrs[b][l])
        waves, mode, cap = C.c_int(0), C.c_int(0), C.c_int(0)
        args = (self._h, batch, stride, _ptr(n), int(n_bound), _ptr(kps2d), _ptr(kps3d), _ptr(flags), pp, cp, C.byref(cam),
                _ptr(pose_guess), int(dbg_level), C.c_uint32(ws_fill), _ptr(pose_out), _ptr(cost), _ptr(trace), _ptr(dbg),
                C.byref(waves), C.byref(mode), C.byref(cap))
        if mats_out is None:
            _check(lib().svo_sparse_align_batch(*args))
        else:
            assert mats_out.numel() * mats_out.element_size() >= batch * pose_mats_layout()["bytes"]
            _check(lib().svo_sparse_align_batch_mats(*args, _ptr(mats_out)))
        return pose_out, cost, trace, dbg, (waves.value, mode.value, cap.value)

    def sia_records_check(self, n, n_bound, kps2d, flags, prev_pyrs, cam, rec_cap=None, ws_fill=0, want_records=False, want_ref=False):
        batch, stride = kps2d.shape[0], kps2d.shape[1]
        levels = cam.max_pyramid_levels
        if rec_cap is None:
            rec_cap = (max(int(n_bound), 1) + 255) // 256 * 256
        used = levels - cam.min_pyramid_level_pose_estimation
        rec = torch.empty((batch, used, 68, rec_cap), dtype=torch.float32, device=kps2d.device) if want_records else None
        ref = torch.empty((batch, used, 68, rec_cap), dtype=torch.float32, device=kps2d.device) if want_ref else None
        pp = (Image * (batch * levels))()
        for b in range(batch):
            for l in range(levels):
                pp[b * levels + l] = _img(prev_pyrs[b][l])
        n_diff, first = C.c_int64(0), C.c_int64(0)
        _check(lib().svo_sia_records_check(self._h, batch, stride, _ptr(n), int(n_bound), _ptr(kps2d), _ptr(flags), pp,
                                           C.byref(cam), int(rec_cap), C.c_uint32(ws_fill), _ptr(rec), _ptr(ref), C.byref(n_diff),
                                           C.byref(first)))
        return (n_diff.value, first.value, rec, ref) if want_ref else (n_diff.value, first.value, rec)

    def project_keypoints(self, pose, kps3d, cam):
        n = kps3d.shape[0]
        out = torch.zeros((n, 2), dtype=torch.float32, device=kps3d.device)
        _check(lib().svo_project_keypoints(self._h, _ptr(pose), _ptr(kps3d), n, C.byref(cam), _ptr(out)))
        return out

    def klt_track(self, prev_lk, cur_lk, prev_pts, cur_pts, win):
        n = prev_pts.shape[0]
        dev = prev_pts.device
        status = torch.zeros(n, dtype=torch.uint8, device=dev)
        err = torch.zeros(n, dtype=torch.float32, device=dev)
        nl = min(len(prev_lk), len(cur_lk))
        _check(lib().svo_klt_track(self._h, _imgs(prev_lk), _imgs(cur_lk), nl, _ptr(prev_pts),
                                   _ptr(cur_pts), n, win, _ptr(status), _ptr(err)))
        return cur_pts, status, err

    def klt_track_batch(self, seqs, n_bound, win, use_mats):
        arr = (KltSequence * len(seqs))()
        keep = []
        for b, s in enumerate(seqs):
            kfs = (KltKeyframe * len(s["kfs"]))()
            keep.append(kfs)
            for k, f in enumerate(s["kfs"]):
                for l, im in enumerate(f["lk"]):
                    kfs[k].lk[l] = _img(im)
                tm, va = f.get("tmpl"), f.get("valid")
                kfs[k].n_lk, kfs[k].n_kps, kfs[k].kps2d = len(f["lk"]), f["kps2d"].shape[0], _ptr(f["kps2d"])
                kfs[k].tmpl, kfs[k].tmpl_valid = _ptr(tm), _ptr(va)
                kfs[k].tmpl_bytes = 0 if tm is None else tm.numel() * tm.element_size()
                kfs[k].tmpl_valid_bytes = 0 if va is None else va.numel() * va.element_size()
                kfs[k].tmpl_cap, kfs[k].tmpl_win = int(f.get("tmpl_cap", 0)), int(f.get("tmpl_win", 0))
            a = arr[b]
            a.kfs, a.n_kfs, a.n_cur = kfs, len(s["kfs"]), len(s["cur"])
            for l, im in enumerate(s["cur"]):
                a.cur[l] = _img(im)
            assert s["n"].dtype == torch.int32 and s["kp_index"].dtype == torch.int32
            assert s.get("kf_id") is None or s["kf_id"].dtype == torch.int32
            a.n, a.kf_id, a.kp_index, a.kps3d, a.pose = (_ptr(s["n"]), _ptr(s.get("kf_id")), _ptr(s["kp_index"]),
                                                         _ptr(s["kps3d"]), _ptr(s["pose"]))
            a.cam = s["cam"]
            a.tracked, a.status, a.err, a.proj_out, a.ref_out = (_ptr(s["tracked"]), _ptr(s["status"]), _ptr(s["err"]),
                                                                 _ptr(s["proj_out"]), _ptr(s.get("ref_out")))
        _check(lib().svo_klt_track_batch(self._h, len(seqs), arr, int(n_bound), int(win), int(bool(use_mats))))

    def pinv6_check(self, H, impl):
        n = H.shape[0]
        out = torch.empty((n, 114), dtype=torch.float32, device=H.device)
        sweeps = torch.empty(n, dtype=torch.int32, device=H.device)
        _check(lib().svo_pinv6_check(self._h, _ptr(H), n, _ptr(out), _ptr(sweeps), int(impl)))
        return out, sweeps

    def solve6_check(self, H, b, impl):
        n = H.shape[0]
        out = torch.empty((n, 120), dtype=torch.float32, device=H.device)
        sweeps = torch.empty(n, dtype=torch.int32, device=H.device)
        _check(lib().svo_solve6_check(self._h, _ptr(H), _ptr(b), n, _ptr(out), _ptr(sweeps), int(impl)))
        return out, sweeps

    def reproj_gn(self, kps2d, kps3d, flags, cam, pose_in, tracked=None, err=None):
        dev = kps2d.device
        n = kps2d.shape[0]
        pose_out = torch.zeros(6, dtype=torch.float32, device=dev)
        cost = torch.zeros(1, dtype=torch.float32, device=dev)
        trace = torch.zeros(GN_TRACE_DTYPE.itemsize, dtype=torch.uint8, device=dev)
        _check(lib().svo_reproj_gn(self._h, _ptr(kps2d), _ptr(kps3d), _ptr(flags), n, C.byref(cam),
                                   _ptr(tracked), _ptr(err), _ptr(pose_in), _ptr(pose_out),
                                   _ptr(cost), _ptr(trace)))
        return pose_out, cost, trace

    def reproj_gn_batch(self, n, n_bound, kps2d, kps3d, flags, cam, pose_in, tracked=None, err=None, zero_out=None):
        batch, stride = kps2d.shape[0], kps2d.shape[1]
        dev = kps2d.device
        pose_out = torch.zeros((batch, 6), dtype=torch.float32, device=dev)
        cost = torch.zeros(batch, dtype=torch.float32, device=dev)
        trace = torch.zeros((batch, GN_TRACE_DTYPE.itemsize), dtype=torch.uint8, device=dev)
        waves, cap = C.c_int(0), C.c_int(0)
        _check(lib().svo_reproj_gn_batch(self._h, batch, stride, _ptr(n), int(n_bound), _ptr(kps2d), _ptr(kps3d),
                                         _ptr(flags), C.byref(cam), _ptr(tracked), _ptr(err), _ptr(pose_in),
                                         _ptr(pose_out), _ptr(cost), _ptr(trace), _ptr(zero_out), C.byref(waves),
                                         C.byref(cap)))
        return pose_out, cost, trace, waves.value, cap.value

    def ssd_disparity(self, left, right, kps2d, win, search_x, search_y, clamp_half=1):
        n = kps2d.shape[0]
        out = torch.zeros(n, dtype=torch.float32, device=kps2d.device)
        a, b = _img(left), _img(right)
        _check(lib().svo_ssd_disparity(self._h, C.byref(a), C.byref(b), _ptr(kps2d), n, win,
                                       search_x, search_y, clamp_half, _ptr(out)))
        return out

    def depth_filter_update(self, kps2d, kps3d, flags, cam, frame_pose, disparity, ref3d, ref2d,
                            kf_pose, outlier, inlier, kf_x, kf_p, do_outlier_check=1, do_update=1):
        n = kps2d.shape[0]
        _check(lib().svo_depth_filter_update(
            self._h, _ptr(kps2d), _ptr(kps3d), _ptr(flags), n, C.byref(cam), _ptr(frame_pose),
            _ptr(disparity), _ptr(ref3d), _ptr(ref2d), _ptr(kf_pose), _ptr(outlier), _ptr(inlier),
            _ptr(kf_x), _ptr(kf_p), do_outlier_check, do_update))

    def filter_update_batch(self, n, n_bound, kps2d, kps3d, flags, cam, frame_pose, disparity, ref3d, ref2d, kf_pose,
                            outlier, inlier, kf_x, kf_p, do_outlier_check, do_update, do_flags, do_reproject, width,
                            height, inside_count):
        batch, stride = kps2d.shape[0], kps2d.shape[1]
        _check(lib().svo_filter_update_batch(
            self._h, batch, stride, _ptr(n), int(n_bound), _ptr(kps2d), _ptr(kps3d), _ptr(flags), C.byref(cam),
            _ptr(frame_pose), _ptr(disparity), _ptr(ref3d), _ptr(ref2d), _ptr(kf_pose), _ptr(outlier), _ptr(inlier),
            _ptr(kf_x), _ptr(kf_p), int(do_outlier_check), int(do_update), int(do_flags), int(do_reproject),
            int(width), int(height), _ptr(inside_count)))

    def filter_update_table_batch(self, seqs, n_bound, do_outlier_check=1, do_update=1, do_flags=1, do_reproject=1):
        arr = (FilterTableSequence * len(seqs))()
        keep = []
        for a, s in zip(arr, seqs):
            kfs = (FilterKeyframe * max(len(s["kfs"]), 1))()
            keep.append(kfs)
            for k, f in zip(kfs, s["kfs"]):
                _fill(k, f, skip=("pose",))
                k.pose[:] = [float(v) for v in f["pose"]]
            _fill(a, s, skip=("kfs", "table"))
            a.kfs, a.table = kfs, int(s.get("table", len(s["kfs"])))
        _check(lib().svo_filter_update_table_batch(self._h, len(seqs), arr, int(n_bound), int(do_outlier_check),
                                                   int(do_update), int(do_flags), int(do_reproject)))

    def compact_batch(self, seqs, cap):
        arr = (CompactSequence * len(seqs))()
        for a, s in zip(arr, seqs):
            _fill(a, s)
        threads = C.c_int(0)
        _check(lib().svo_compact_batch(self._h, len(seqs), arr, int(cap), C.byref(threads)))
        return threads.value

    def keyframe_merge_batch(self, seqs, n_levels, max_cells, cap):
        arr = (MergeSequence * len(seqs))()
        for a, s in zip(arr, seqs):
            _fill(a, s)
        threads = C.c_int(0)
        _check(lib().svo_keyframe_merge_batch(self._h, len(seqs), arr, int(n_levels), int(max_cells), int(cap),
                                              C.byref(threads)))
        return threads.value

    def keyframe_init_batch(self, seqs, cap):
        arr = (KfInitSequence * len(seqs))()
        for a, s in zip(arr, seqs):
            _fill(a, s)
        _check(lib().svo_keyframe_init_batch(self._h, len(seqs), arr, int(cap)))

    def ssd_disparity_batch(self, seqs, n_bound, win, search_y):
        arr = (SsdSequence * len(seqs))()
        for a, s in zip(arr, seqs):
            _fill(a, s, skip=("left", "right"))
            a.left, a.right = _img(s["left"]), _img(s["right"])
        max_win = C.c_int(0)
        _check(lib().svo_ssd_disparity_batch(self._h, len(seqs), arr, int(n_bound), int(win), int(search_y),
                                             C.byref(max_win)))
        return max_win.value


def detect_to_numpy(cells, counts):
    c = cells.cpu().numpy().view(DET_CELL_DTYPE)[..., 0]
    return [c[l, :k].copy() for l, k in enumerate(counts.cpu().numpy())]


def trace_to_numpy(t):
    return t.cpu().numpy().view(GN_TRACE_DTYPE)
```

Baseline: 293,600.

## Rewrite SSD disparity kernel as a single-wave block with register prefix sums

Rewrites the stereo SSD disparity kernel to run one 64-lane wave per keypoint instead of a 256-thread block. All MFMA cross-correlation tiles are kept in one wave's registers, column energies are computed in registers, and DPP wave scans build prefix sums, replacing the shared-memory window sums and block barriers. Global loads are batched so they are issued before edge handling. A reference kernel and a check entry point are added to compare results. This trades block-level parallelism for fewer barriers, less LDS traffic and higher occupancy, at the cost of more registers per lane and more serial work per wave.

```diff
diff --git a/include/svo_hip.h b/include/svo_hip.h
--- a/include/svo_hip.h
+++ b/include/svo_hip.h
@@ -947,6 +947,9 @@
 } svo_ssd_sequence;
 int svo_ssd_disparity_batch(svo_handle *h, int batch, const svo_ssd_sequence *seqs, int n_bound, int win, int search_y,
                             int *max_win);
+int svo_ssd_disparity_check(svo_handle *h, int batch, const svo_ssd_sequence *seqs, int n_bound, int win, int search_y,
+                            int stride, uint32_t fill, float *disp_out, float *ref_out, int64_t *n_diff,
+                            int64_t *first_diff);
 
 typedef struct svo_filter_keyframe {
     float pose[6];
diff --git a/stereo-svo-slam_amd/csrc/depth.hip b/stereo-svo-slam_amd/csrc/depth.hip
--- a/stereo-svo-slam_amd/csrc/depth.hip
+++ b/stereo-svo-slam_amd/csrc/depth.hip
@@ -1,69 +1,97 @@
-#include "svo_kernels.hpp"
+#include "ssd_common.hpp"
 
 namespace svo {
 
-typedef uint32_t __attribute__((aligned(1))) u32_unaligned;
-__device__ inline uint32_t load_u8x4(const ImgView& im, int y, int x, int valid) {
-    const uint8_t* src = im.g() + (size_t)y * im.stride + x;
-    uint32_t v;
-    if (x + 4 <= im.w) {
-        v = *reinterpret_cast<const u32_unaligned*>(src);
+constexpr int SSD_P_STRIDE = 100;
+
+__device__ __forceinline__ void ssd_wave_sync() {
+    __builtin_amdgcn_fence(__ATOMIC_RELEASE, "wavefront");
+    __builtin_amdgcn_wave_barrier();
+    __builtin_amdgcn_fence(__ATOMIC_ACQUIRE, "wavefront");
+}
+
+__device__ __forceinline__ int ssd_wave_scan_i(int v) {
+    v += __builtin_amdgcn_update_dpp(0, v, 0x111, 0xF, 0xF, false);
+    v += __builtin_amdgcn_update_dpp(0, v, 0x112, 0xF, 0xF, false);
+    v += __builtin_amdgcn_update_dpp(0, v, 0x114, 0xF, 0xF, false);
+    v += __builtin_amdgcn_update_dpp(0, v, 0x118, 0xF, 0xF, false);
+    v += __builtin_amdgcn_update_dpp(0, v, 0x142, 0xA, 0xF, false);
+    v += __builtin_amdgcn_update_dpp(0, v, 0x143, 0xC, 0xF, false);
+    return v;
+}
+
+template <int R_ROWS, int N_MB, int N_JB, int NMB, int NJB>
+__device__ __forceinline__ void ssd_cross(const uint8_t* s_t, const uint8_t* s_r, int th, int lane, ssd_v4i (&acc)[N_MB][N_JB]) {
+    const int fm = lane & 15, fh = lane >> 4;
+    const int o = 16 + 16 * fh - fm;
+    const uint32_t* tb = reinterpret_cast<const uint32_t*>(s_t) + (o >> 2);
+    const unsigned sh = (unsigned)(o & 3);
+    const uint8_t* ab = s_r + 16 * fh;
+    struct Row { uint32_t t[5]; ssd_v4i af[NMB][NJB]; };
+    auto read_row = [&](int r, Row& w) {
+        const uint32_t* t = tb + r * (SSD_T_STRIDE / 4);
+#pragma unroll
+        for (int d = 0; d < 5; d++) w.t[d] = t[d];
+#pragma unroll
+        for (int mb = 0; mb < NMB; mb++)
+#pragma unroll
+            for (int jb = 0; jb < NJB; jb++)
+                w.af[mb][jb] = *reinterpret_cast<const ssd_v4i*>(ab + 16 * jb + min(16 * mb + fm + r, R_ROWS - 1) * SSD_R_STRIDE);
+    };
+    auto use_row = [&](const Row& w) {
+        ssd_v4i bf;
+        bf.x = (int)__builtin_amdgcn_alignbyte(w.t[1], w.t[0], sh);
+        bf.y = (int)__builtin_amdgcn_alignbyte(w.t[2], w.t[1], sh);
+        bf.z = (int)__builtin_amdgcn_alignbyte(w.t[3], w.t[2], sh);
+        bf.w = (int)__builtin_amdgcn_alignbyte(w.t[4], w.t[3], sh);
+#pragma unroll
+        for (int mb = 0; mb < NMB; mb++)
+#pragma unroll
+            for (int jb = 0; jb < NJB; jb++)
+                acc[mb][jb] = __builtin_amdgcn_mfma_i32_16x16x64_i8(w.af[mb][jb], bf, acc[mb][jb], 0, 0, 0);
+    };
+    if constexpr (NMB * NJB <= 5) {
+        for (int r = 0; r < th; r += 2) {
+            Row r0, r1;
+            read_row(r, r0);
+            read_row(r + 1, r1);
+            use_row(r0);
+            use_row(r1);
+        }
     } else {
-        v = 0;
-#pragma unroll
-        for (int b = 0; b < 4; b++)
-            if (x + b < im.w) v |= (uint32_t)src[b] << (8 * b);
-    }
-    if (valid < 4) v &= (1u << (8 * valid)) - 1u;
-    return v;
-}
-
-__device__ inline uint4 load_u8x16(const ImgView& im, int y, int x, int valid, uint32_t flip, uint32_t pad) {
-    uint32_t w[4];
-    if (x + 16 <= im.w) {
-        const uint8_t* src = im.g() + (size_t)y * im.stride + x;
-        __builtin_memcpy(w, src, 16);
-    } else {
-#pragma unroll
-        for (int k = 0; k < 4; k++) w[k] = load_u8x4(im, y, x + 4 * k, 4);
-    }
-#pragma unroll
-    for (int k = 0; k < 4; k++) {
-        const int nv = valid - 4 * k;
-        const uint32_t vm = nv >= 4 ? 0xFFFFFFFFu : (nv <= 0 ? 0u : ((1u << (8 * nv)) - 1u));
-        w[k] = ((w[k] ^ flip) & vm) | (pad & ~vm);
-    }
-    return make_uint4(w[0], w[1], w[2], w[3]);
-}
-
-constexpr int SSD_WIN_ALL = 35, SSD_MH_ALL = 17;
-constexpr int SSD_MAX_MW = 65;
-constexpr int SSD_T_STRIDE = 96;
-constexpr int SSD_R_STRIDE = 144;
-constexpr int SSD_W_STRIDE = 105;
-#ifndef SVO_SSD_THREADS
-#define SVO_SSD_THREADS 256
-#endif
-constexpr int SSD_THREADS = SVO_SSD_THREADS;
-
-typedef int ssd_v4i __attribute__((ext_vector_type(4)));
+        for (int r = 0; r < th; r++) {
+            Row cur;
+            read_row(r, cur);
+            use_row(cur);
+        }
+    }
+}
+template <int R_ROWS, int N_MB, int N_JB, int NMB>
+__device__ __forceinline__ void ssd_cross_jb(const uint8_t* s_t, const uint8_t* s_r, int th, int lane, int n_jb,
+                                             ssd_v4i (&acc)[N_MB][N_JB]) {
+    static_assert(N_JB == 5, "one case per column block count");
+    switch (n_jb) {
+        case 1: ssd_cross<R_ROWS, N_MB, N_JB, NMB, 1>(s_t, s_r, th, lane, acc); break;
+        case 2: ssd_cross<R_ROWS, N_MB, N_JB, NMB, 2>(s_t, s_r, th, lane, acc); break;
+        case 3: ssd_cross<R_ROWS, N_MB, N_JB, NMB, 3>(s_t, s_r, th, lane, acc); break;
+        case 4: ssd_cross<R_ROWS, N_MB, N_JB, NMB, 4>(s_t, s_r, th, lane, acc); break;
+        default: ssd_cross<R_ROWS, N_MB, N_JB, NMB, 5>(s_t, s_r, th, lane, acc); break;
+    }
+}
 
 template <int SSD_MAX_WIN, int SSD_MAX_MH>
-__global__ __launch_bounds__(SSD_THREADS) void ssd_disparity_kernel(const SsdArgs* __restrict__ args) {
-    constexpr int SSD_R_ROWS = SSD_MAX_WIN + SSD_MAX_MH, SSD_MAX_MATCH = SSD_MAX_MW * SSD_MAX_MH;
+__global__ __launch_bounds__(64) __attribute__((amdgpu_waves_per_eu(4))) void ssd_disparity_kernel(const SsdArgs* __restrict__ args) {
+    constexpr int SSD_R_ROWS = SSD_MAX_WIN + SSD_MAX_MH, SSD_T_ROWS = SSD_MAX_WIN + 1;
+    constexpr int N_MB = (SSD_MAX_MH + 15) / 16, N_JB = (SSD_MAX_MW + 15) / 16;
     const SsdArgs& a = args[blockIdx.y];
     if (a.enable && !*G(a.enable)) return;
     const int n = *G(a.n_ptr);
     const int kp = a.first + (a.first_ptr ? *G(a.first_ptr) : 0) + (int)blockIdx.x;
     if (kp >= n) return;
-    const int tid = threadIdx.x, lane = tid & 63, wave = tid >> 6;
-
-    __shared__ __attribute__((aligned(16))) uint8_t s_t[(SSD_MAX_WIN + 1) * SSD_T_STRIDE];
+    const int lane = threadIdx.x;
+
+    __shared__ __attribute__((aligned(16))) uint8_t s_t[SSD_T_ROWS * SSD_T_STRIDE];
     __shared__ __attribute__((aligned(16))) uint8_t s_r[SSD_R_ROWS * SSD_R_STRIDE];
-    __shared__ int s_w[SSD_MAX_MH * SSD_W_STRIDE];
-    __shared__ int s_tt[4];
-    __shared__ unsigned long long s_key[SSD_THREADS / 64];
-    __shared__ int s_sum[SSD_THREADS / 64], s_cnt[SSD_THREADS / 64];
 
     const int window_before = a.win / 2, window_after = (a.win + 1) / 2;
     const int cols = a.left.w, rows = a.left.h;
@@ -83,160 +111,175 @@
     if (a.clamp_half && (x12 <= 0 || y12 <= 0 || x11 >= cols - 1 || y11 >= rows - 1)) skip = true;
     if (a.clamp_half && (x22 <= 0 || y22 <= 0 || x21 >= cols - 1 || y21 >= rows - 1)) skip = true;
     if (tw <= 0 || th <= 0 || mw <= 0 || mh <= 0) skip = true;
-    if (tw > SSD_MAX_WIN || th > SSD_MAX_WIN || mw > SSD_MAX_MW || mh > SSD_MAX_MH || rw > SSD_W_STRIDE ||
+    if (tw > SSD_MAX_WIN || th > SSD_MAX_WIN || mw > SSD_MAX_MW || mh > SSD_MAX_MH || rw >= SSD_P_STRIDE ||
         rh > SSD_R_ROWS)
         skip = true;
     if (skip) {
-        if (tid == 0) G(a.disparity)[kp] = -1.0f;
+        if (lane == 0) G(a.disparity)[kp] = -1.0f;
         return;
     }
 
     static_assert(SSD_T_STRIDE % 16 == 0 && SSD_R_STRIDE % 16 == 0, "rows are whole 16-byte chunks");
-    for (int i = tid; i < (SSD_MAX_WIN + 1) * (SSD_T_STRIDE / 16); i += SSD_THREADS) {
-        const int r = i / (SSD_T_STRIDE / 16), ch = i % (SSD_T_STRIDE / 16);
-        const int c = 16 * (ch - 1);
-        uint4 v = make_uint4(0, 0, 0, 0);
-        if (r < th && c >= 0 && c < tw) v = load_u8x16(a.left, y11 + r, x11 + c, tw - c, 0x80808080u, 0u);
-        reinterpret_cast<uint4*>(s_t)[i] = v;
-    }
-    for (int i = tid; i < SSD_R_ROWS * (SSD_R_STRIDE / 16); i += SSD_THREADS) {
-        const int r = i / (SSD_R_STRIDE / 16), ch = i % (SSD_R_STRIDE / 16);
-        uint4 v = make_uint4(0, 0, 0, 0);
-        if (r < rh && 16 * ch < rw) v = load_u8x16(a.right, y21 + r, x21 + 16 * ch, rw - 16 * ch, 0x80808080u, 0x80808080u);
-        reinterpret_cast<uint4*>(s_r)[i] = v;
-    }
-    __syncthreads();
-
-    if (wave == SSD_THREADS / 64 - 1) {
-        int tt = 0;
-        if (lane < th) {
-            const uint32_t* trow = reinterpret_cast<const uint32_t*>(s_t + lane * SSD_T_STRIDE) + 4;
-#pragma unroll
-            for (int d = 0; d < 9; d++) tt = __builtin_amdgcn_sdot4((int)trow[d], (int)trow[d], tt, false);
-        }
-        tt = wave_sum_dpp_i(tt);
-        if (lane == 0) s_tt[0] = tt;
-    }
-    if (tid < rw) {
-        const int8_t* col = reinterpret_cast<const int8_t*>(s_r) + tid;
-        int sq = 0;
-        for (int r = 0; r < th; r++) {
-            const int v = col[r * SSD_R_STRIDE];
-            sq += __mul24(v, v);
-        }
-        s_w[tid] = sq;
-        for (int k = 1; k < mh; k++) {
-            const int vn = col[(k + th - 1) * SSD_R_STRIDE], vo = col[(k - 1) * SSD_R_STRIDE];
-            sq += __mul24(vn, vn) - __mul24(vo, vo);
-            s_w[k * SSD_W_STRIDE + tid] = sq;
-        }
-    }
-
-    const int n_jb = (mw + 15) >> 4, n_mb = (mh + 15) >> 4;
+    {
+        constexpr int T_CH = SSD_T_STRIDE / 16, R_CH = SSD_R_STRIDE / 16;
+        constexpr int NT = SSD_T_ROWS * T_CH, NR = SSD_R_ROWS * R_CH, T_TRIPS = (NT + 63) / 64, R_TRIPS = (NR + 63) / 64;
+        uint4 tv[T_TRIPS], rv[R_TRIPS];
+        const int lw = a.left.w, rwid = a.right.w;
+#pragma unroll
+        for (int t = 0; t < T_TRIPS; t++) {
+            const int i = lane + 64 * t, r = i / T_CH, c = 16 * (i % T_CH - 1);
+            tv[t] = make_uint4(0, 0, 0, 0);
+            if (r < th && c >= 0 && c < tw && x11 + c + 16 <= lw) tv[t] = load_u8x16_whole(a.left, y11 + r, x11 + c);
+        }
+#pragma unroll
+        for (int t = 0; t < R_TRIPS; t++) {
+            const int i = lane + 64 * t, r = i / R_CH, c = 16 * (i % R_CH);
+            rv[t] = make_uint4(0, 0, 0, 0);
+            if (r < rh && c < rw && x21 + c + 16 <= rwid) rv[t] = load_u8x16_whole(a.right, y21 + r, x21 + c);
+        }
+#pragma unroll
+        for (int t = 0; t < T_TRIPS; t++) {
+            const int i = lane + 64 * t, r = i / T_CH, c = 16 * (i % T_CH - 1);
+            if (r < th && c >= 0 && c < tw && x11 + c + 16 > lw) tv[t] = load_u8x16_edge(a.left, y11 + r, x11 + c);
+        }
+#pragma unroll
+        for (int t = 0; t < R_TRIPS; t++) {
+            const int i = lane + 64 * t, r = i / R_CH, c = 16 * (i % R_CH);
+            if (r < rh && c < rw && x21 + c + 16 > rwid) rv[t] = load_u8x16_edge(a.right, y21 + r, x21 + c);
+        }
+#pragma unroll
+        for (int t = 0; t < T_TRIPS; t++) {
+            const int i = lane + 64 * t, r = i / T_CH, c = 16 * (i % T_CH - 1);
+            uint4 v = make_uint4(0, 0, 0, 0);
+            if (r < th && c >= 0 && c < tw) v = finish_u8x16(tv[t], tw - c, 0x80808080u, 0u);
+            if (NT % 64 == 0 || i < NT) reinterpret_cast<uint4*>(s_t)[i] = v;
+        }
+#pragma unroll
+        for (int t = 0; t < R_TRIPS; t++) {
+            const int i = lane + 64 * t, r = i / R_CH, c = 16 * (i % R_CH);
+            uint4 v = make_uint4(0, 0, 0, 0);
+            if (r < rh && c < rw) v = finish_u8x16(rv[t], rw - c, 0x80808080u, 0x80808080u);
+            if (NR % 64 == 0 || i < NR) reinterpret_cast<uint4*>(s_r)[i] = v;
+        }
+    }
+    ssd_wave_sync();
+
+    int stt = 0;
+    if (lane < th) {
+        const uint32_t* trow = reinterpret_cast<const uint32_t*>(s_t + lane * SSD_T_STRIDE) + 4;
+#pragma unroll
+        for (int d = 0; d < 9; d++) stt = __builtin_amdgcn_sdot4((int)trow[d], (int)trow[d], stt, false);
+    }
+    stt = wave_sum_dpp_i(stt);
+
+    const int n_jb = (mw + 15) >> 4;
     const int fm = lane & 15, fh = lane >> 4;
-    constexpr int SSD_SLOTS = (10 + SSD_THREADS / 64 - 1) / (SSD_THREADS / 64);
-    ssd_v4i acc[SSD_SLOTS];
-    int task_of[SSD_SLOTS];
-#pragma unroll
-    for (int t = 0; t < SSD_SLOTS; t++) { acc[t] = ssd_v4i{0, 0, 0, 0}; task_of[t] = -1; }
+    ssd_v4i acc[N_MB][N_JB];
+#pragma unroll
+    for (int mb = 0; mb < N_MB; mb++)
+#pragma unroll
+        for (int jb = 0; jb < N_JB; jb++) acc[mb][jb] = ssd_v4i{0, 0, 0, 0};
+    static_assert(N_MB <= 2, "two row blocks of 16 at most");
+    if (N_MB == 2 && mh > 16) ssd_cross_jb<SSD_R_ROWS, N_MB, N_JB, N_MB>(s_t, s_r, th, lane, n_jb, acc);
+    else ssd_cross_jb<SSD_R_ROWS, N_MB, N_JB, 1>(s_t, s_r, th, lane, n_jb, acc);
+    int w0[SSD_MAX_MH], w1[SSD_MAX_MH];
     {
-        int slot = 0;
-        for (int task = wave; task < n_jb * n_mb && slot < SSD_SLOTS; task += SSD_THREADS / 64, slot++) {
-            task_of[slot] = task;
-            const int mb = task >= n_jb ? 1 : 0, jb = task - mb * n_jb;
-            const int o = 16 + 16 * fh - fm;
-            const uint32_t* tb = reinterpret_cast<const uint32_t*>(s_t) + (o >> 2);
-            const unsigned sh = (unsigned)(o & 3);
-            const uint8_t* ab = s_r + (16 * jb + 16 * fh);
-            const int arow = 16 * mb + fm;
-            ssd_v4i c = {0, 0, 0, 0};
-            for (int r = 0; r < th; r++) {
-                const uint32_t* t = tb + r * (SSD_T_STRIDE / 4);
-                const uint32_t t0 = t[0], t1 = t[1], t2 = t[2], t3 = t[3], t4 = t[4];
-                ssd_v4i bf;
-                bf.x = (int)__builtin_amdgcn_alignbyte(t1, t0, sh);
-                bf.y = (int)__builtin_amdgcn_alignbyte(t2, t1, sh);
-                bf.z = (int)__builtin_amdgcn_alignbyte(t3, t2, sh);
-                bf.w = (int)__builtin_amdgcn_alignbyte(t4, t3, sh);
-                const ssd_v4i af = *reinterpret_cast<const ssd_v4i*>(ab + min(arow + r, SSD_R_ROWS - 1) * SSD_R_STRIDE);
-                c = __builtin_amdgcn_mfma_i32_16x16x64_i8(af, bf, c, 0, 0, 0);
-            }
-            acc[slot] = c;
-        }
-    }
-    __syncthreads();
-
-    static_assert(sizeof(int) * SSD_MAX_MATCH <= SSD_R_ROWS * SSD_R_STRIDE, "match map must fit the region tile");
-    static_assert(SSD_MAX_MH <= 32, "two row blocks of 16 at most");
-    int* const s_m = reinterpret_cast<int*>(s_r);
-    {
-        const int seg_len = (mw + 7) >> 3;
-        for (int item = tid; item < mh * 8; item += SSD_THREADS) {
-            const int k = item >> 3, j0 = (item & 7) * seg_len, j1 = min(mw, j0 + seg_len);
-            if (j0 < j1) {
-                const int* wrow = &s_w[k * SSD_W_STRIDE];
-                int sq = 0;
-                for (int c = 0; c < tw; c++) sq += wrow[j0 + c];
-                s_m[k * mw + j0] = sq;
-                for (int j = j0 + 1; j < j1; j++) {
-                    sq += wrow[j + tw - 1] - wrow[j - 1];
-                    s_m[k * mw + j] = sq;
+        const int8_t* col = reinterpret_cast<const int8_t*>(s_r) + lane;
+        int sq0 = 0, sq1 = 0;
+        for (int r0 = 0; r0 < th; r0 += 8) {
+            int v0[8], v1[8];
+#pragma unroll
+            for (int i = 0; i < 8; i++) {
+                const int rr = min(r0 + i, SSD_R_ROWS - 1);
+                v0[i] = col[rr * SSD_R_STRIDE];
+                v1[i] = col[rr * SSD_R_STRIDE + 64];
+            }
+#pragma unroll
+            for (int i = 0; i < 8; i++) {
+                const bool in = r0 + i < th;
+                sq0 += in ? __mul24(v0[i], v0[i]) : 0;
+                sq1 += in ? __mul24(v1[i], v1[i]) : 0;
+            }
+        }
+        w0[0] = sq0; w1[0] = sq1;
+        const int8_t* coln = col + (th - 1) * SSD_R_STRIDE;
+        int n0[SSD_MAX_MH], n1[SSD_MAX_MH], o0[SSD_MAX_MH], o1[SSD_MAX_MH];
+#pragma unroll
+        for (int k = 1; k < SSD_MAX_MH; k++) {
+            n0[k] = coln[k * SSD_R_STRIDE]; n1[k] = coln[k * SSD_R_STRIDE + 64];
+            o0[k] = col[(k - 1) * SSD_R_STRIDE]; o1[k] = col[(k - 1) * SSD_R_STRIDE + 64];
+        }
+#pragma unroll
+        for (int k = 1; k < SSD_MAX_MH; k++) {
+            sq0 += __mul24(n0[k], n0[k]) - __mul24(o0[k], o0[k]);
+            sq1 += __mul24(n1[k], n1[k]) - __mul24(o1[k], o1[k]);
+            w0[k] = sq0; w1[k] = sq1;
+        }
+    }
+    ssd_wave_sync();
+
+    static_assert(sizeof(int) * SSD_MAX_MH * SSD_P_STRIDE <= SSD_R_ROWS * SSD_R_STRIDE, "the prefix rows must fit the region tile");
+    static_assert(SSD_MAX_WIN + SSD_MAX_MW <= SSD_P_STRIDE && SSD_P_STRIDE <= 128 + 1, "a row holds rw + 1 prefixes of two columns per lane");
+    int* const s_p = reinterpret_cast<int*>(s_r);
+#pragma unroll
+    for (int k = 0; k < SSD_MAX_MH; k++) {
+        if (k < mh) {
+            const int p0 = ssd_wave_scan_i(w0[k]);
+            const int p1 = ssd_wave_scan_i(w1[k]) + __builtin_amdgcn_readlane(p0, 63);
+            if (lane == 0) s_p[k * SSD_P_STRIDE] = 0;
+            if (lane < rw) s_p[k * SSD_P_STRIDE + lane + 1] = p0;
+            if (lane + 64 < rw) s_p[k * SSD_P_STRIDE + lane + 65] = p1;
+        }
+    }
+    ssd_wave_sync();
+
+    unsigned long long best = ~0ull;
+#pragma unroll
+    for (int mb = 0; mb < N_MB; mb++)
+#pragma unroll
+        for (int jb = 0; jb < N_JB; jb++) {
+            if (jb < n_jb && 16 * mb < mh) {
+                const int j = 16 * jb + fm, jc = min(j, mw - 1);
+#pragma unroll
+                for (int i = 0; i < 4; i++) {
+                    const int k = 16 * mb + 4 * fh + i, kc = min(k, SSD_MAX_MH - 1);
+                    const int* prow = &s_p[kc * SSD_P_STRIDE + jc];
+                    const int ssd = prow[tw] - prow[0] + stt - 2 * acc[mb][jb][i];
+                    const float f = (float)ssd;
+                    acc[mb][jb][i] = (int)__float_as_uint(f);
+                    if (k < mh && j < mw) {
+                        const unsigned long long key = ((unsigned long long)__float_as_uint(f) << 32) | (unsigned)(k * mw + j);
+                        best = key < best ? key : best;
+                    }
                 }
             }
         }
-    }
-    __syncthreads();
-    {
-        const int stt = s_tt[0];
-#pragma unroll
-        for (int slot = 0; slot < SSD_SLOTS; slot++) {
-            const int task = task_of[slot];
-            if (task < 0) continue;
-            const int mb = task >= n_jb ? 1 : 0, jb = task - mb * n_jb;
-            const int j = 16 * jb + fm;
-#pragma unroll
-            for (int i = 0; i < 4; i++) {
-                const int k = 16 * mb + 4 * fh + i;
-                if (k < mh && j < mw) s_m[k * mw + j] += stt - 2 * acc[slot][i];
-            }
-        }
-    }
-    __syncthreads();
-
-    const int nm = mw * mh;
-    unsigned long long best = ~0ull;
-    for (int o = tid; o < nm; o += SSD_THREADS) {
-        const unsigned long long key = ((unsigned long long)__float_as_uint((float)s_m[o]) << 32) | (unsigned)o;
-        best = key < best ? key : best;
-    }
 #pragma unroll
     for (int o = 32; o >= 1; o >>= 1) {
         const unsigned long long other = __shfl_xor(best, o, 64);
         best = other < best ? other : best;
     }
-    if ((tid & 63) == 0) s_key[tid >> 6] = best;
-    __syncthreads();
-    best = s_key[0];
-    for (int w = 1; w < SSD_THREADS / 64; w++) best = s_key[w] < best ? s_key[w] : best;
-    const int min_o = (int)(best & 0xffffffffu);
+    const int min_o = __builtin_amdgcn_readfirstlane((int)(best & 0xffffffffu));
     const int minx = min_o % mw, miny = min_o / mw;
-    const float minVal = __uint_as_float((unsigned)(best >> 32));
+    const float minVal = __uint_as_float((unsigned)__builtin_amdgcn_readfirstlane((int)(best >> 32)));
 
     int sumj = 0, cnt = 0;
-    const unsigned magic = ((1u << 20) + (unsigned)mw - 1u) / (unsigned)mw;
-    for (int o = tid; o < nm; o += SSD_THREADS) {
-        const int k = (int)(((unsigned)o * magic) >> 20), j = o - k * mw;
-        if (j >= minx && k >= miny && (double)(float)s_m[o] <= (double)minVal) { sumj += j; cnt++; }
-    }
+#pragma unroll
+    for (int mb = 0; mb < N_MB; mb++)
+#pragma unroll
+        for (int jb = 0; jb < N_JB; jb++) {
+            const int j = 16 * jb + fm;
+#pragma unroll
+            for (int i = 0; i < 4; i++) {
+                const int k = 16 * mb + 4 * fh + i;
+                if (k < mh && j < mw && j >= minx && k >= miny && (double)__uint_as_float((unsigned)acc[mb][jb][i]) <= (double)minVal) { sumj += j; cnt++; }
+            }
+        }
     sumj = wave_sum_dpp_i(sumj);
     cnt = wave_sum_dpp_i(cnt);
-    if ((tid & 63) == 0) { s_sum[tid >> 6] = sumj; s_cnt[tid >> 6] = cnt; }
-    __syncthreads();
-    if (tid == 0) {
-        int ts = 0, tc = 0;
-        for (int w = 0; w < SSD_THREADS / 64; w++) { ts += s_sum[w]; tc += s_cnt[w]; }
-        float minPos = (float)ts;
-        minPos = minPos / tc;
+    if (lane == 0) {
+        float minPos = (float)sumj;
+        minPos = minPos / cnt;
         G(a.disparity)[kp] = a.clamp_half ? fmaxf(0.5f, minPos) : minPos;
     }
 }
@@ -245,10 +288,14 @@
 
 void launch_ssd(const SsdArgs* d_args, int batch, int max_n, int win, int search_y, hipStream_t stream) {
     if (max_n <= 0) return;
+#ifdef SVO_SSD_FOUR_WAVES
+    launch_ssd_ref(d_args, batch, max_n, win, search_y, stream);
+    return;
+#endif
     if (ssd_pick_max_win(win, search_y) == 31)
-        hipLaunchKernelGGL((ssd_disparity_kernel<31, 13>), dim3(max_n, batch), dim3(SSD_THREADS), 0, stream, d_args);
+        hipLaunchKernelGGL((ssd_disparity_kernel<31, 13>), dim3(max_n, batch), dim3(64), 0, stream, d_args);
     else
-        hipLaunchKernelGGL((ssd_disparity_kernel<SSD_WIN_ALL, SSD_MH_ALL>), dim3(max_n, batch), dim3(SSD_THREADS), 0, stream, d_args);
+        hipLaunchKernelGGL((ssd_disparity_kernel<SSD_WIN_ALL, SSD_MH_ALL>), dim3(max_n, batch), dim3(64), 0, stream, d_args);
 }
 
 __global__ __launch_bounds__(64) void filter_update_kernel(const FilterArgs* __restrict__ args) {
diff --git a/stereo-svo-slam_amd/csrc/ssd_common.hpp b/stereo-svo-slam_amd/csrc/ssd_common.hpp
--- /dev/null
+++ b/stereo-svo-slam_amd/csrc/ssd_common.hpp
@@ -0,0 +1,57 @@
+#pragma once
+#include "svo_kernels.hpp"
+
+namespace svo {
+
+typedef uint32_t __attribute__((aligned(1))) u32_unaligned;
+__device__ inline uint32_t load_u8x4(const ImgView& im, int y, int x, int valid) {
+    const uint8_t* src = im.g() + (size_t)y * im.stride + x;
+    uint32_t v;
+    if (x + 4 <= im.w) {
+        v = *reinterpret_cast<const u32_unaligned*>(src);
+    } else {
+        v = 0;
+#pragma unroll
+        for (int b = 0; b < 4; b++)
+            if (x + b < im.w) v |= (uint32_t)src[b] << (8 * b);
+    }
+    if (valid < 4) v &= (1u << (8 * valid)) - 1u;
+    return v;
+}
+
+__device__ inline uint4 load_u8x16_whole(const ImgView& im, int y, int x) {
+    uint32_t w[4];
+    const uint8_t* src = im.g() + (size_t)y * im.stride + x;
+    __builtin_memcpy(w, src, 16);
+    return make_uint4(w[0], w[1], w[2], w[3]);
+}
+__device__ inline uint4 load_u8x16_edge(const ImgView& im, int y, int x) {
+    uint32_t w[4];
+#pragma unroll
+    for (int k = 0; k < 4; k++) w[k] = load_u8x4(im, y, x + 4 * k, 4);
+    return make_uint4(w[0], w[1], w[2], w[3]);
+}
+__device__ inline uint4 finish_u8x16(uint4 raw, int valid, uint32_t flip, uint32_t pad) {
+    uint32_t w[4] = {raw.x, raw.y, raw.z, raw.w};
+#pragma unroll
+    for (int k = 0; k < 4; k++) {
+        const int nv = valid - 4 * k;
+        const uint32_t vm = nv >= 4 ? 0xFFFFFFFFu : (nv <= 0 ? 0u : ((1u << (8 * nv)) - 1u));
+        w[k] = ((w[k] ^ flip) & vm) | (pad & ~vm);
+    }
+    return make_uint4(w[0], w[1], w[2], w[3]);
+}
+__device__ inline uint4 load_u8x16(const ImgView& im, int y, int x, int valid, uint32_t flip, uint32_t pad) {
+    return finish_u8x16(x + 16 <= im.w ? load_u8x16_whole(im, y, x) : load_u8x16_edge(im, y, x), valid, flip, pad);
+}
+
+constexpr int SSD_WIN_ALL = 35, SSD_MH_ALL = 17;
+constexpr int SSD_MAX_MW = 65;
+constexpr int SSD_T_STRIDE = 96;
+constexpr int SSD_R_STRIDE = 144;
+
+typedef int ssd_v4i __attribute__((ext_vector_type(4)));
+
+void launch_ssd_ref(const SsdArgs* d_args, int batch, int max_n, int win, int search_y, hipStream_t stream);
+
+}
diff --git a/stereo-svo-slam_amd/csrc/svo_capi_check.hip b/stereo-svo-slam_amd/csrc/svo_capi_check.hip
--- a/stereo-svo-slam_amd/csrc/svo_capi_check.hip
+++ b/stereo-svo-slam_amd/csrc/svo_capi_check.hip
@@ -5,6 +5,7 @@
 #include <cstring>
 #include <vector>
 
+#include "ssd_common.hpp"
 #include "svo_handle.hpp"
 
 using namespace svo;
@@ -765,31 +766,30 @@
     return finish_launch(h);
 }
 
-extern "C" int svo_ssd_disparity_batch(svo_handle* h, int batch, const svo_ssd_sequence* seqs, int n_bound, int win,
-                                       int search_y, int* max_win) {
-    CHECK_H(h);
+static int ssd_fill_blocks(const char* who, svo_handle* h, int batch, const svo_ssd_sequence* seqs, int n_bound, int win,
+                           int search_y, bool own_disparity, std::vector<SsdArgs>& blocks) {
     constexpr int kMaxIndex = 1 << 29;
     if (bad_batch(batch, seqs) || n_bound < 0 || n_bound > kMaxIndex)
-        return svo_set_error(SVO_ERR_INVALID, "svo_ssd_disparity_batch: need 1 <= batch <= 4096, seqs and 0 <= n_bound <= 2^29");
+        return svo_set_error(SVO_ERR_INVALID, "%s: need 1 <= batch <= 4096, seqs and 0 <= n_bound <= 2^29", who);
     if (win < 1 || win > 35 || search_y < 0 || search_y > 8)
-        return svo_set_error(SVO_ERR_INVALID, "svo_ssd_disparity_batch: win<=35, search_y<=8 supported");
+        return svo_set_error(SVO_ERR_INVALID, "%s: win<=35, search_y<=8 supported", who);
     HIP_TRY(hipStreamSynchronize(h->stream));
-    std::vector<SsdArgs> blocks((size_t)batch);
+    blocks.resize((size_t)batch);
     for (int b = 0; b < batch; b++) {
         const svo_ssd_sequence& s = seqs[b];
-        if (klt_bad_view(s.left) || klt_bad_view(s.right) || !s.n || s.cap < 0 || (s.cap > 0 && (!s.kps2d || !s.disparity)) ||
-            s.first < 0 || s.first > kMaxIndex)
-            return svo_set_error(SVO_ERR_INVALID, "svo_ssd_disparity_batch: sequence %d: bad arguments", b);
+        if (klt_bad_view(s.left) || klt_bad_view(s.right) || !s.n || s.cap < 0 ||
+            (s.cap > 0 && (!s.kps2d || (own_disparity && !s.disparity))) || s.first < 0 || s.first > kMaxIndex)
+            return svo_set_error(SVO_ERR_INVALID, "%s: sequence %d: bad arguments", who, b);
         if (s.win < 1 || s.win > win || s.search_x < 0 || s.search_x > 64 || s.search_y < 0 || s.search_y > search_y)
-            return svo_set_error(SVO_ERR_INVALID, "svo_ssd_disparity_batch: sequence %d: win %d, search_x %d, search_y %d exceed "
-                                 "the launch's %d, 64, %d", b, s.win, s.search_x, s.search_y, win, search_y);
+            return svo_set_error(SVO_ERR_INVALID, "%s: sequence %d: win %d, search_x %d, search_y %d exceed "
+                                 "the launch's %d, 64, %d", who, b, s.win, s.search_x, s.search_y, win, search_y);
         int32_t n = 0, first = 0;
         if (const int rc = read_i32(s.n, 1, &n)) return rc;
         if (s.first_ptr)
             if (const int rc = read_i32(s.first_ptr, 1, &first)) return rc;
         if (n < 0 || n > s.cap || first < 0 || first > kMaxIndex)
-            return svo_set_error(SVO_ERR_INVALID, "svo_ssd_disparity_batch: sequence %d: n = %d is outside 0..cap = %d, or "
-                                 "*first_ptr = %d is outside 0..2^29", b, n, s.cap, first);
+            return svo_set_error(SVO_ERR_INVALID, "%s: sequence %d: n = %d is outside 0..cap = %d, or "
+                                 "*first_ptr = %d is outside 0..2^29", who, b, n, s.cap, first);
         SsdArgs& sa = blocks[(size_t)b];
         memset(&sa, 0, sizeof(sa));
         sa.left = make_view(s.left); sa.right = make_view(s.right);
@@ -798,12 +798,272 @@
         sa.first = s.first; sa.first_ptr = s.first_ptr;
         sa.enable = s.enable;
     }
+    return SVO_OK;
+}
+
+extern "C" int svo_ssd_disparity_batch(svo_handle* h, int batch, const svo_ssd_sequence* seqs, int n_bound, int win,
+                                       int search_y, int* max_win) {
+    CHECK_H(h);
+    std::vector<SsdArgs> blocks;
+    int rc = ssd_fill_blocks("svo_ssd_disparity_batch", h, batch, seqs, n_bound, win, search_y, true, blocks);
+    if (rc) return rc;
     SsdArgs* d;
-    const int rc = stage(h, blocks, &d);
+    rc = stage(h, blocks, &d);
     if (rc) return rc;
     if (max_win) *max_win = ssd_pick_max_win(win, search_y);
     launch_ssd(d, batch, n_bound, win, search_y, h->stream);
     return finish_launch(h);
+}
+
+constexpr int SSD_W_STRIDE = 105;
+constexpr int SSD_REF_THREADS = 256;
+
+template <int SSD_MAX_WIN, int SSD_MAX_MH>
+__global__ __launch_bounds__(SSD_REF_THREADS) void ssd_disparity_ref_kernel(const SsdArgs* __restrict__ args) {
+    constexpr int SSD_THREADS = SSD_REF_THREADS;
+    constexpr int SSD_R_ROWS = SSD_MAX_WIN + SSD_MAX_MH, SSD_MAX_MATCH = SSD_MAX_MW * SSD_MAX_MH;
+    const SsdArgs& a = args[blockIdx.y];
+    if (a.enable && !*G(a.enable)) return;
+    const int n = *G(a.n_ptr);
+    const int kp = a.first + (a.first_ptr ? *G(a.first_ptr) : 0) + (int)blockIdx.x;
+    if (kp >= n) return;
+    const int tid = threadIdx.x, lane = tid & 63, wave = tid >> 6;
+
+    __shared__ __attribute__((aligned(16))) uint8_t s_t[(SSD_MAX_WIN + 1) * SSD_T_STRIDE];
+    __shared__ __attribute__((aligned(16))) uint8_t s_r[SSD_R_ROWS * SSD_R_STRIDE];
+    __shared__ int s_w[SSD_MAX_MH * SSD_W_STRIDE];
+    __shared__ int s_tt[4];
+    __shared__ unsigned long long s_key[SSD_THREADS / 64];
+    __shared__ int s_sum[SSD_THREADS / 64], s_cnt[SSD_THREADS / 64];
+
+    const int window_before = a.win / 2, window_after = (a.win + 1) / 2;
+    const int cols = a.left.w, rows = a.left.h;
+    const svo_kp2d p = G(a.kps2d)[kp];
+    const int x = (int)p.x, y = (int)p.y;
+    const int x11 = max(0, x - window_before);
+    const int x12 = min(cols - 1, x + window_after);
+    const int y11 = max(0, y - window_before);
+    const int y12 = min(rows, y + window_after);
+    const int x21 = x11;
+    const int x22 = min(cols - 1, x + window_after + a.search_x);
+    const int y21 = max(0, y - window_before - a.search_y);
+    const int y22 = min(rows - 1, y + window_after + a.search_y);
+    const int tw = x12 - x11, th = y12 - y11, rw = x22 - x21, rh = y22 - y21;
+    const int mw = rw - tw + 1, mh = rh - th + 1;
+    bool skip = false;
+    if (a.clamp_half && (x12 <= 0 || y12 <= 0 || x11 >= cols - 1 || y11 >= rows - 1)) skip = true;
+    if (a.clamp_half && (x22 <= 0 || y22 <= 0 || x21 >= cols - 1 || y21 >= rows - 1)) skip = true;
+    if (tw <= 0 || th <= 0 || mw <= 0 || mh <= 0) skip = true;
+    if (tw > SSD_MAX_WIN || th > SSD_MAX_WIN || mw > SSD_MAX_MW || mh > SSD_MAX_MH || rw > SSD_W_STRIDE ||
+        rh > SSD_R_ROWS)
+        skip = true;
+    if (skip) {
+        if (tid == 0) G(a.disparity)[kp] = -1.0f;
+        return;
+    }
+
+    static_assert(SSD_T_STRIDE % 16 == 0 && SSD_R_STRIDE % 16 == 0, "rows are whole 16-byte chunks");
+    for (int i = tid; i < (SSD_MAX_WIN + 1) * (SSD_T_STRIDE / 16); i += SSD_THREADS) {
+        const int r = i / (SSD_T_STRIDE / 16), ch = i % (SSD_T_STRIDE / 16);
+        const int c = 16 * (ch - 1);
+        uint4 v = make_uint4(0, 0, 0, 0);
+        if (r < th && c >= 0 && c < tw) v = load_u8x16(a.left, y11 + r, x11 + c, tw - c, 0x80808080u, 0u);
+        reinterpret_cast<uint4*>(s_t)[i] = v;
+    }
+    for (int i = tid; i < SSD_R_ROWS * (SSD_R_STRIDE / 16); i += SSD_THREADS) {
+        const int r = i / (SSD_R_STRIDE / 16), ch = i % (SSD_R_STRIDE / 16);
+        uint4 v = make_uint4(0, 0, 0, 0);
+        if (r < rh && 16 * ch < rw) v = load_u8x16(a.right, y21 + r, x21 + 16 * ch, rw - 16 * ch, 0x80808080u, 0x80808080u);
+        reinterpret_cast<uint4*>(s_r)[i] = v;
+    }
+    __syncthreads();
+
+    if (wave == SSD_THREADS / 64 - 1) {
+        int tt = 0;
+        if (lane < th) {
+            const uint32_t* trow = reinterpret_cast<const uint32_t*>(s_t + lane * SSD_T_STRIDE) + 4;
+#pragma unroll
+            for (int d = 0; d < 9; d++) tt = __builtin_amdgcn_sdot4((int)trow[d], (int)trow[d], tt, false);
+        }
+        tt = wave_sum_dpp_i(tt);
+        if (lane == 0) s_tt[0] = tt;
+    }
+    if (tid < rw) {
+        const int8_t* col = reinterpret_cast<const int8_t*>(s_r) + tid;
+        int sq = 0;
+        for (int r = 0; r < th; r++) {
+            const int v = col[r * SSD_R_STRIDE];
+            sq += __mul24(v, v);
+        }
+        s_w[tid] = sq;
+        for (int k = 1; k < mh; k++) {
+            const int vn = col[(k + th - 1) * SSD_R_STRIDE], vo = col[(k - 1) * SSD_R_STRIDE];
+            sq += __mul24(vn, vn) - __mul24(vo, vo);
+            s_w[k * SSD_W_STRIDE + tid] = sq;
+        }
+    }
+
+    const int n_jb = (mw + 15) >> 4, n_mb = (mh + 15) >> 4;
+    const int fm = lane & 15, fh = lane >> 4;
+    constexpr int SSD_SLOTS = (10 + SSD_THREADS / 64 - 1) / (SSD_THREADS / 64);
+    ssd_v4i acc[SSD_SLOTS];
+    int task_of[SSD_SLOTS];
+#pragma unroll
+    for (int t = 0; t < SSD_SLOTS; t++) { acc[t] = ssd_v4i{0, 0, 0, 0}; task_of[t] = -1; }
+    {
+        int slot = 0;
+        for (int task = wave; task < n_jb * n_mb && slot < SSD_SLOTS; task += SSD_THREADS / 64, slot++) {
+            task_of[slot] = task;
+            const int mb = task >= n_jb ? 1 : 0, jb = task - mb * n_jb;
+            const int o = 16 + 16 * fh - fm;
+            const uint32_t* tb = reinterpret_cast<const uint32_t*>(s_t) + (o >> 2);
+            const unsigned sh = (unsigned)(o & 3);
+            const uint8_t* ab = s_r + (16 * jb + 16 * fh);
+            const int arow = 16 * mb + fm;
+            ssd_v4i c = {0, 0, 0, 0};
+            for (int r = 0; r < th; r++) {
+                const uint32_t* t = tb + r * (SSD_T_STRIDE / 4);
+                const uint32_t t0 = t[0], t1 = t[1], t2 = t[2], t3 = t[3], t4 = t[4];
+                ssd_v4i bf;
+                bf.x = (int)__builtin_amdgcn_alignbyte(t1, t0, sh);
+                bf.y = (int)__builtin_amdgcn_alignbyte(t2, t1, sh);
+                bf.z = (int)__builtin_amdgcn_alignbyte(t3, t2, sh);
+                bf.w = (int)__builtin_amdgcn_alignbyte(t4, t3, sh);
+                const ssd_v4i af = *reinterpret_cast<const ssd_v4i*>(ab + min(arow + r, SSD_R_ROWS - 1) * SSD_R_STRIDE);
+                c = __builtin_amdgcn_mfma_i32_16x16x64_i8(af, bf, c, 0, 0, 0);
+            }
+            acc[slot] = c;
+        }
+    }
+    __syncthreads();
+
+    static_assert(sizeof(int) * SSD_MAX_MATCH <= SSD_R_ROWS * SSD_R_STRIDE, "match map must fit the region tile");
+    static_assert(SSD_MAX_MH <= 32, "two row blocks of 16 at most");
+    int* const s_m = reinterpret_cast<int*>(s_r);
+    {
+        const int seg_len = (mw + 7) >> 3;
+        for (int item = tid; item < mh * 8; item += SSD_THREADS) {
+            const int k = item >> 3, j0 = (item & 7) * seg_len, j1 = min(mw, j0 + seg_len);
+            if (j0 < j1) {
+                const int* wrow = &s_w[k * SSD_W_STRIDE];
+                int sq = 0;
+                for (int c = 0; c < tw; c++) sq += wrow[j0 + c];
+                s_m[k * mw + j0] = sq;
+                for (int j = j0 + 1; j < j1; j++) {
+                    sq += wrow[j + tw - 1] - wrow[j - 1];
+                    s_m[k * mw + j] = sq;
+                }
+            }
+        }
+    }
+    __syncthreads();
+    {
+        const int stt = s_tt[0];
+#pragma unroll
+        for (int slot = 0; slot < SSD_SLOTS; slot++) {
+            const int task = task_of[slot];
+            if (task < 0) continue;
+            const int mb = task >= n_jb ? 1 : 0, jb = task - mb * n_jb;
+            const int j = 16 * jb + fm;
+#pragma unroll
+            for (int i = 0; i < 4; i++) {
+                const int k = 16 * mb + 4 * fh + i;
+                if (k < mh && j < mw) s_m[k * mw + j] += stt - 2 * acc[slot][i];
+            }
+        }
+    }
+    __syncthreads();
+
+    const int nm = mw * mh;
+    unsigned long long best = ~0ull;
+    for (int o = tid; o < nm; o += SSD_THREADS) {
+        const unsigned long long key = ((unsigned long long)__float_as_uint((float)s_m[o]) << 32) | (unsigned)o;
+        best = key < best ? key : best;
+    }
+#pragma unroll
+    for (int o = 32; o >= 1; o >>= 1) {
+        const unsigned long long other = __shfl_xor(best, o, 64);
+        best = other < best ? other : best;
+    }
+    if ((tid & 63) == 0) s_key[tid >> 6] = best;
+    __syncthreads();
+    best = s_key[0];
+    for (int w = 1; w < SSD_THREADS / 64; w++) best = s_key[w] < best ? s_key[w] : best;
+    const int min_o = (int)(best & 0xffffffffu);
+    const int minx = min_o % mw, miny = min_o / mw;
+    const float minVal = __uint_as_float((unsigned)(best >> 32));
+
+    int sumj = 0, cnt = 0;
+    const unsigned magic = ((1u << 20) + (unsigned)mw - 1u) / (unsigned)mw;
+    for (int o = tid; o < nm; o += SSD_THREADS) {
+        const int k = (int)(((unsigned)o * magic) >> 20), j = o - k * mw;
+        if (j >= minx && k >= miny && (double)(float)s_m[o] <= (double)minVal) { sumj += j; cnt++; }
+    }
+    sumj = wave_sum_dpp_i(sumj);
+    cnt = wave_sum_dpp_i(cnt);
+    if ((tid & 63) == 0) { s_sum[tid >> 6] = sumj; s_cnt[tid >> 6] = cnt; }
+    __syncthreads();
+    if (tid == 0) {
+        int ts = 0, tc = 0;
+        for (int w = 0; w < SSD_THREADS / 64; w++) { ts += s_sum[w]; tc += s_cnt[w]; }
+        float minPos = (float)ts;
+        minPos = minPos / tc;
+        G(a.disparity)[kp] = a.clamp_half ? fmaxf(0.5f, minPos) : minPos;
+    }
+}
+
+void svo::launch_ssd_ref(const SsdArgs* d_args, int batch, int max_n, int win, int search_y, hipStream_t stream) {
+    if (max_n <= 0) return;
+    if (ssd_pick_max_win(win, search_y) == 31)
+        hipLaunchKernelGGL((ssd_disparity_ref_kernel<31, 13>), dim3(max_n, batch), dim3(SSD_REF_THREADS), 0, stream, d_args);
+    else
+        hipLaunchKernelGGL((ssd_disparity_ref_kernel<SSD_WIN_ALL, SSD_MH_ALL>), dim3(max_n, batch), dim3(SSD_REF_THREADS), 0, stream, d_args);
+}
+
+extern "C" int svo_ssd_disparity_check(svo_handle* h, int batch, const svo_ssd_sequence* seqs, int n_bound, int win,
+                                       int search_y, int stride, uint32_t fill, float* disp_out, float* ref_out,
+                                       int64_t* n_diff, int64_t* first_diff) {
+    CHECK_H(h);
+    if (!n_diff || !first_diff || stride < 1)
+        return svo_set_error(SVO_ERR_INVALID, "svo_ssd_disparity_check: need n_diff, first_diff and stride >= 1");
+    std::vector<SsdArgs> blocks;
+    int rc = ssd_fill_blocks("svo_ssd_disparity_check", h, batch, seqs, n_bound, win, search_y, false, blocks);
+    if (rc) return rc;
+    for (int b = 0; b < batch; b++)
+        if (seqs[b].cap > stride)
+            return svo_set_error(SVO_ERR_INVALID, "svo_ssd_disparity_check: sequence %d: cap %d exceeds stride %d", b, seqs[b].cap, stride);
+    const size_t words = (size_t)batch * (size_t)stride;
+    DevPtr<float> ws;
+    DevPtr<unsigned long long> res;
+    HIP_TRY(dev_malloc(ws, sizeof(float) * 2 * words));
+    HIP_TRY(dev_malloc(res, 2 * sizeof(unsigned long long)));
+    HIP_TRY(hipMemsetD32Async(reinterpret_cast<hipDeviceptr_t>(ws.get()), (int)fill, 2 * words, h->stream));
+    const unsigned long long init[2] = {0ull, ~0ull};
+    HIP_TRY(hipMemcpyAsync(res.get(), init, sizeof(init), hipMemcpyHostToDevice, h->stream));
+    blocks.resize((size_t)2 * batch);
+    for (int b = 0; b < batch; b++) {
+        blocks[(size_t)b].disparity = ws.get() + (size_t)b * stride;
+        blocks[(size_t)(batch + b)] = blocks[(size_t)b];
+        blocks[(size_t)(batch + b)].disparity = ws.get() + words + (size_t)b * stride;
+    }
+    SsdArgs* d;
+    rc = stage(h, blocks, &d);
+    if (rc) return rc;
+    launch_ssd(d, batch, n_bound, win, search_y, h->stream);
+    HIP_TRY(hipGetLastError());
+    launch_ssd_ref(d + batch, batch, n_bound, win, search_y, h->stream);
+    HIP_TRY(hipGetLastError());
+    words_diff_kernel<<<(unsigned)std::min<size_t>((words + 255) / 256, 1024), 256, 0, h->stream>>>(
+        reinterpret_cast<const uint32_t*>(ws.get()), reinterpret_cast<const uint32_t*>(ws.get() + words), words, res.get());
+    HIP_TRY(hipGetLastError());
+    if (disp_out) HIP_TRY(hipMemcpyAsync(disp_out, ws.get(), sizeof(float) * words, hipMemcpyDeviceToDevice, h->stream));
+    if (ref_out) HIP_TRY(hipMemcpyAsync(ref_out, ws.get() + words, sizeof(float) * words, hipMemcpyDeviceToDevice, h->stream));
+    unsigned long long got[2];
+    HIP_TRY(hipMemcpyAsync(got, res.get(), sizeof(got), hipMemcpyDeviceToHost, h->stream));
+    HIP_TRY(hipStreamSynchronize(h->stream));
+    *n_diff = (int64_t)got[0];
+    *first_diff = got[0] ? (int64_t)got[1] : -1;
+    return SVO_OK;
 }
 
 static_assert(sizeof(svo_filter_keyframe) == 72 && sizeof(svo_filter_table_sequence) == 248, "the layouts the Python binding restates");
diff --git a/stereo-svo-slam_amd/stereo_svo_slam_amd/hip_lib.py b/stereo-svo-slam_amd/stereo_svo_slam_amd/hip_lib.py
--- a/stereo-svo-slam_amd/stereo_svo_slam_amd/hip_lib.py
+++ b/stereo-svo-slam_amd/stereo_svo_slam_amd/hip_lib.py
@@ -55,7 +55,7 @@
     "svo_keyframe_launch_info", "svo_compact_batch", "svo_keyframe_merge_batch", "svo_keyframe_init_batch",
     "svo_keyframe_record_layout", "svo_ssd_disparity_batch",
     "svo_sparse_align_batch_mats", "svo_pose_mats_layout", "svo_filter_update_table_batch",
-    "svo_sia_records_check",
+    "svo_sia_records_check", "svo_ssd_disparity_check",
 )
 
 INPUT_GRAY_PAIR, INPUT_BGR_PAIR, INPUT_RGB_PAIR, INPUT_SBS_GRAY, INPUT_SBS_BGR, INPUT_SBS_RGB, INPUT_CH3_ECON = range(7)
@@ -1408,6 +1408,18 @@
                                              C.byref(max_win)))
         return max_win.value
 
+    def ssd_disparity_check(self, seqs, n_bound, win, search_y, stride, fill=0):
+        arr = (SsdSequence * len(seqs))()
+        for a, s in zip(arr, seqs):
+            _fill(a, s, skip=("left", "right"))
+            a.left, a.right = _img(s["left"]), _img(s["right"])
+        out = torch.empty((len(seqs), int(stride)), dtype=torch.float32, device=self.device)
+        ref = torch.empty_like(out)
+        n_diff, first = C.c_int64(0), C.c_int64(0)
+        _check(lib().svo_ssd_disparity_check(self._h, len(seqs), arr, int(n_bound), int(win), int(search_y), int(stride),
+                                             C.c_uint32(fill), _ptr(out), _ptr(ref), C.byref(n_diff), C.byref(first)))
+        return n_diff.value, first.value, out, ref
+
 
 def detect_to_numpy(cells, counts):
     c = cells.cpu().numpy().view(DET_CELL_DTYPE)[..., 0]
```

Result: faster. 326,800, median of 6 (+11.3%).
